# learner-shx/SVG-IR

Hardware: AMD Instinct MI355X
Metric: Gaussian-surfels/sec fwd+bwd @800x800 (1 view) (higher is better)
Workload: dtype f32; 1 GPU; cfg2: rgss path, P=200000 surfels, 800x800, SH degree 3, S=5, VS=0, fwd+bwd, one view per step per GPU (BASELINE.json configs[1] = cfg2 at N=1; configs[3] = cfg4, view r on rank r, at N>1); num_rendered=673008, parallelism=view-parallel x1, per_rank_cpus=not pinned

## Files before the change

### svg-ir_amd/csrc/api.hip

```cpp
#include <algorithm>
#include <cstdarg>
#include <cstdio>
#include <atomic>
#include <cstdlib>
#include <ctime>
#include <memory>
#include <mutex>
#include <string>
#include <vector>

#include "common.hpp"
#include "geom_bwd.hpp"
#include "workload_history.hpp"
#include "depth_sort_plan.hpp"

using namespace svgir;

namespace {

thread_local std::string g_err;
std::atomic<bool> g_prof{false};
WorkloadHistory g_history;
unsigned long long* pinned_words(size_t n) {
    void* ptr = nullptr;
    if (hipHostMalloc(&ptr, n * sizeof(unsigned long long), hipHostMallocCoherent) != hipSuccess) { (void)hipGetLastError(); return nullptr; }
    std::fill_n((unsigned long long*)ptr, n, 0ull);
    return (unsigned long long*)ptr;
}
unsigned long long* g_pinned = nullptr;
std::atomic<uint32_t> g_pinned_tag{0};
constexpr unsigned kPinnedSlots = 256;
std::once_flag g_pinned_once;
std::mutex g_pinned_mu;
uint64_t g_pinned_busy[kPinnedSlots / 64];
struct PinnedSlot {
    unsigned long long* at = nullptr; uint32_t tag = 0; int index = -1;
    PinnedSlot() {
        std::call_once(g_pinned_once, [] { g_pinned = pinned_words(2 * kPinnedSlots); });
        tag = ++g_pinned_tag;
        if (tag == 0) tag = ++g_pinned_tag;
        if (!g_pinned) return;
        static const unsigned usable = [] { const char* e = getenv("SVGIR_PINNED_SLOTS"); return e ? (unsigned)std::min<long>(std::max<long>(atol(e), 0), kPinnedSlots) : kPinnedSlots; }();
        std::lock_guard<std::mutex> lk(g_pinned_mu);
        for (unsigned i = 0; i < usable; i++)
            if (!(g_pinned_busy[i / 64] >> (i % 64) & 1ull)) {
                g_pinned_busy[i / 64] |= 1ull << (i % 64);
                index = (int)i;
                at = g_pinned + 2 * index;
                return;
            }
    }
    ~PinnedSlot() {
        if (index < 0) return;
        std::lock_guard<std::mutex> lk(g_pinned_mu);
        g_pinned_busy[index / 64] &= ~(1ull << (index % 64));
    }
    PinnedSlot(const PinnedSlot&) = delete;
    PinnedSlot& operator=(const PinnedSlot&) = delete;
};
double spin_budget_s() {
    static const double v = [] {
        const char* e = getenv("SVGIR_SPIN_MS");
        return e ? std::max(0.0, atof(e)) * 1e-3 : 0.05;
    }();
    return v;
}
inline bool tagged_pair(volatile unsigned long long* at, uint32_t tag, uint32_t* w0, uint32_t* w1) {
    const unsigned long long v0 = at[0], v1 = at[1];
    if ((uint32_t)(v0 >> 32) != tag || (uint32_t)(v1 >> 32) != tag) return false;
    *w0 = (uint32_t)v0; *w1 = (uint32_t)v1;
    return true;
}
bool pinned_spin(volatile unsigned long long* at, uint32_t tag, uint32_t* w0, uint32_t* w1) {
    struct timespec t0;
    clock_gettime(CLOCK_MONOTONIC, &t0);
    const double budget = spin_budget_s();
    for (long long spin = 0;; spin++) {
        if (tagged_pair(at, tag, w0, w1)) return true;
        if ((spin & 255) == 255 || budget == 0.0) {
            struct timespec t1;
            clock_gettime(CLOCK_MONOTONIC, &t1);
            const double el = (double)(t1.tv_sec - t0.tv_sec) + 1e-9 * (double)(t1.tv_nsec - t0.tv_nsec);
            if (el >= budget) return false;
            if (el > 5e-3) { struct timespec ts = {0, 20000}; nanosleep(&ts, nullptr); }
        }
    }
}
struct ViewEntry { const void* key = nullptr; uint32_t tag = 0; int cap_R = 0; long long cap_slots = -1; unsigned long long stamp = 0;
                   bool queue = false;
                   bool recorded = false;
                   hipStream_t stream = nullptr; };
constexpr int kViewEntries = 1024;
std::mutex g_view_mu;
ViewEntry g_view[kViewEntries];
constexpr int kViewWords = 4;
unsigned long long* g_view_pinned = nullptr;
unsigned long long g_view_clock = 0;
uint32_t g_view_tag = 0;
unsigned long long* view_note(const void* image_blob, int cap_R, long long cap_slots, bool queue, uint32_t* tag, hipStream_t stream) {
    std::lock_guard<std::mutex> lk(g_view_mu);
    if (!g_view_pinned && !(g_view_pinned = pinned_words(kViewEntries * kViewWords))) return nullptr;
    int slot = 0;
    for (int i = 0; i < kViewEntries; i++) {
        if (g_view[i].key == image_blob) { slot = i; break; }
        if (g_view[i].stamp < g_view[slot].stamp) slot = i;
    }
    ViewEntry& e = g_view[slot];
    e.key = image_blob; e.stamp = ++g_view_clock; e.cap_R = cap_R; e.cap_slots = cap_slots; e.recorded = false;
    e.stream = stream; e.queue = queue;
    e.tag = ++g_view_tag ? g_view_tag : ++g_view_tag;
    *tag = e.tag;
    return g_view_pinned + kViewWords * slot;
}
constexpr uint32_t kBlobMagic = 0x53564931u, kBlobMagicQueue = 0x53564932u;
struct ViewCounts { bool known = false; bool queue = false; int cap_R = 0; long long cap_slots = -1, pairs = -1, slots = -1, nonempty = -1; hipError_t err = hipSuccess; };
enum class Wait { kCaps, kLook, kBlock };
ViewCounts resolve_view(const void* image_blob, const uint32_t* blob_counters, Wait how, const hipStream_t* stream, bool caps = false,
                        const CapKey* record = nullptr) {
    ViewCounts out;
    if (!image_blob) return out;
    int i = 0;
    uint32_t tag = 0;
    hipStream_t fwd_stream = nullptr;
    {
        std::lock_guard<std::mutex> lk(g_view_mu);
        while (g_view_pinned && i < kViewEntries && g_view[i].key != image_blob) i++;
        if (!g_view_pinned || i == kViewEntries) i = -1;
        else { tag = g_view[i].tag; fwd_stream = g_view[i].stream; out.cap_R = g_view[i].cap_R; out.cap_slots = g_view[i].cap_slots; out.queue = g_view[i].queue; }
    }
    out.known = i >= 0;
    if (out.known && how != Wait::kCaps) {
        volatile unsigned long long* at = g_view_pinned + kViewWords * i;
        uint32_t w0 = 0, w1 = 0;
        bool got = how == Wait::kLook ? tagged_pair(at, tag, &w0, &w1) : pinned_spin(at, tag, &w0, &w1);
        if (!got && how == Wait::kBlock) {
            hipError_t e = hipErrorInvalidHandle;
            if (stream) e = hipStreamSynchronize(*stream);
            else {
                const hipError_t q = fwd_stream ? hipStreamQuery(fwd_stream) : hipSuccess;
                if (q == hipSuccess || q == hipErrorNotReady) e = hipStreamSynchronize(fwd_stream);
                else (void)hipGetLastError();
            }
            if (e != hipSuccess) { (void)hipGetLastError(); e = hipDeviceSynchronize(); }
            if (e != hipSuccess) (void)hipGetLastError();
            got = tagged_pair(at, tag, &w0, &w1);
        }
        if (got) {
            out.pairs = (long long)w0; out.slots = (long long)w1;
            const unsigned long long v2 = at[2];
            if ((uint32_t)(v2 >> 32) == tag) out.nonempty = (long long)(uint32_t)v2;
            bool first = false;
            if (record) {
                std::lock_guard<std::mutex> lk(g_view_mu);
                if (g_view[i].key == image_blob && !g_view[i].recorded) g_view[i].recorded = first = true;
            }
            if (first) g_history.record_slots(*record, out.slots, out.nonempty);
        }
    }
    if (blob_counters && (!out.known || (caps && out.cap_slots < 0) || (how != Wait::kCaps && out.pairs < 0))) {
        uint32_t w[8] = {0, 0, 0, 0, 0, 0, 0, 0};
        out.err = stream ? hipStreamSynchronize(*stream) : hipDeviceSynchronize();
        const bool read = out.err == hipSuccess && hipMemcpy(w, blob_counters, sizeof(w), hipMemcpyDeviceToHost) == hipSuccess;
        if (out.err == hipSuccess && !read) (void)hipGetLastError();
        if (!read || (w[3] != kBlobMagic && w[3] != kBlobMagicQueue)) return out;
        out.known = true; out.queue = w[3] == kBlobMagicQueue; out.pairs = (long long)w[1]; out.slots = (long long)w[2]; out.cap_R = (int)w[4];
        out.cap_slots = (long long)((unsigned long long)w[5] | ((unsigned long long)w[6] << 32));
    }
    return out;
}
struct SideStream { hipStream_t s = nullptr; bool ok = false; };
std::mutex g_side_mu;
SideStream g_side[16];
hipStream_t side_stream(hipStream_t of) {
    int dev = 0;
    hipDevice_t sd;
    if (of != nullptr && hipStreamGetDevice(of, &sd) == hipSuccess) dev = (int)sd;
    else if (hipGetDevice(&dev) != hipSuccess) return nullptr;
    if (dev < 0 || dev >= 16) return nullptr;
    std::lock_guard<std::mutex> lk(g_side_mu);
    SideStream& ss = g_side[dev];
    if (!ss.ok) {
        int least = 0, greatest = 0;
        (void)hipDeviceGetStreamPriorityRange(&least, &greatest);
        if (hipStreamCreateWithPriority(&ss.s, hipStreamNonBlocking, least) != hipSuccess) return nullptr;
        ss.ok = true;
    }
    return ss.s;
}
std::mutex g_times_mu;
struct Pending { hipEvent_t a, b; const char* name; };
std::vector<Pending> g_pending;
struct Accum { const char* name; double sum_ms; int count; };
std::vector<Accum> g_accum;

int fail(int code, const char* fmt, ...) {
    char buf[512];
    va_list ap;
    va_start(ap, fmt);
    vsnprintf(buf, sizeof(buf), fmt, ap);
    va_end(ap);
    g_err = buf;
    return code;
}

#define HIP_OK(expr)                                                                                   \
    do {                                                                                               \
        hipError_t e_ = (expr);                                                                        \
        if (e_ != hipSuccess) return fail(SVGIR_ERR_HIP, "%s failed: %s", #expr, hipGetErrorString(e_)); \
    } while (0)

void resolve_pending() {
    std::vector<Pending> todo;
    {
        std::lock_guard<std::mutex> lk(g_times_mu);
        todo.swap(g_pending);
    }
    std::vector<hipEvent_t> seen;
    for (auto& p : todo) {
        (void)hipEventSynchronize(p.b);
        float ms = 0.f;
        if (hipEventElapsedTime(&ms, p.a, p.b) == hipSuccess) {
            std::lock_guard<std::mutex> lk(g_times_mu);
            bool found = false;
            for (auto& acc : g_accum)
                if (acc.name == p.name) { acc.sum_ms += ms; acc.count++; found = true; break; }
            if (!found) g_accum.push_back({p.name, (double)ms, 1});
        }
        for (hipEvent_t e : {p.a, p.b}) {
            bool dup = false;
            for (auto x : seen) if (x == e) dup = true;
            if (!dup) seen.push_back(e);
        }
    }
    for (auto e : seen) (void)hipEventDestroy(e);
}

}

namespace svgir {
StageMarks stage_begin(hipStream_t s) {
    StageMarks t{s, g_prof.load(), nullptr};
    if (t.on) {
        if (hipEventCreate(&t.prev) != hipSuccess) t.on = false;
        else (void)hipEventRecord(t.prev, s);
    }
    return t;
}
void stage_mark(StageMarks& t, const char* name) {
    if (!t.on) return;
    hipEvent_t e;
    if (hipEventCreate(&e) != hipSuccess) { t.on = false; return; }
    (void)hipEventRecord(e, t.s);
    {
        std::lock_guard<std::mutex> lk(g_times_mu);
        g_pending.push_back({t.prev, e, name});
    }
    t.prev = e;
}
int report_error(int code, const char* fmt, ...) {
    char buf[512];
    va_list ap;
    va_start(ap, fmt);
    vsnprintf(buf, sizeof(buf), fmt, ap);
    va_end(ap);
    g_err = buf;
    return code;
}
}

namespace {

struct ViewGrid { int W, H, gx, gy, T; };
ViewGrid view_grid(int W, int H) {
    const int gx = (W + TILE - 1) / TILE, gy = (H + TILE - 1) / TILE;
    return {W, H, gx, gy, (int)((long long)gx * gy)};
}

CfgRef cfg_ref(const svgir_params* p) {
    CfgRef c;
    if (p->variant == SVGIR_SVGSS) { c.ptr = p->config; c.len = p->config ? p->config_len : 0; }
    else { c.ptr = nullptr; c.len = -1; }
    return c;
}

constexpr int kListMinP = 400000, kListMinPRows = 50000;

bool high_fill(long long nonempty) {
    static const int forced = [] { const char* e = getenv("SVGIR_FWD_FILL"); return e ? (atoi(e) != 0 ? 1 : 0) : -1; }();
    return forced >= 0 ? forced != 0 : nonempty >= 8192;
}

bool shade_prepass(int Ns) {
    static const int forced = [] { const char* e = getenv("SVGIR_PREPASS"); return e ? (atoi(e) != 0 ? 1 : 0) : -1; }();
    return forced >= 0 ? forced != 0 : Ns >= 128;
}

int validate(const svgir_params* p, bool fwd) {
    if (!p) return fail(SVGIR_ERR_INVALID, "params is NULL");
    if (p->variant != SVGIR_RGSS && p->variant != SVGIR_SVGSS) return fail(SVGIR_ERR_INVALID, "unknown variant %d", p->variant);
    if (p->P < 0 || p->W <= 0 || p->H <= 0) return fail(SVGIR_ERR_INVALID, "bad sizes P=%d W=%d H=%d", p->P, p->W, p->H);
    if (p->P > 40000000) return fail(SVGIR_ERR_INVALID, "P=%d exceeds the supported 40 000 000 Gaussians (32-bit byte offsets into the splat records)", p->P);
    const ViewGrid v = view_grid(p->W, p->H);
    if (v.gx > 1023 || v.gy > 1023 || 4ll * v.gx * v.gy >= (1ll << (32 - SEG_K_BITS)))
        return fail(SVGIR_ERR_INVALID, "image %dx%d exceeds the supported size (at most 1023 tiles per side, %lld tiles in total)",
                    p->W, p->H, (1ll << (32 - SEG_K_BITS)) / 4 - 1);
    if (p->P == 0) return 0;
    if (!p->means3D || !p->viewmatrix || !p->projmatrix || !p->background)
        return fail(SVGIR_ERR_INVALID, "means3D/viewmatrix/projmatrix/background must be provided");
    if (fwd && !p->opacities) return fail(SVGIR_ERR_INVALID, "opacities must be provided");
    if (!p->colors_precomp && !p->shs)
        return fail(SVGIR_ERR_INVALID, "For non-RGB, provide precomputed Gaussian colors!");
    if (p->shs && (p->D < 0 || p->D > 3 || p->M < (p->D + 1) * (p->D + 1)))
        return fail(SVGIR_ERR_INVALID, "SH degree %d needs M >= %d coefficients (M=%d)", p->D, (p->D + 1) * (p->D + 1), p->M);
    if (p->shs && !p->cam_pos) return fail(SVGIR_ERR_INVALID, "cam_pos is required with SHs");
    if (!p->cov3D_precomp && !(p->scales && p->rotations))
        return fail(SVGIR_ERR_INVALID, "provide scales+rotations or cov3D_precomp");
    if (p->S < 0 || (p->S > 0 && !p->features)) return fail(SVGIR_ERR_INVALID, "features missing for S=%d", p->S);
    if (p->variant == SVGIR_SVGSS) {
        if (p->VS < 0 || p->VS % 4 != 0) return fail(SVGIR_ERR_INVALID, "VS=%d must be a non-negative multiple of 4", p->VS);
        if (p->VS > 0 && !p->vfeatures) return fail(SVGIR_ERR_INVALID, "vfeatures missing for VS=%d", p->VS);
        if (!p->patchbbox) return fail(SVGIR_ERR_INVALID, "patchbbox is required for svgss");
        if (p->S > 50 || p->VS / 4 > 20) return fail(SVGIR_ERR_INVALID, "svgss supports S<=50, VS/4<=20 (Q9)");
    } else {
        if (p->VS != 0) return fail(SVGIR_ERR_INVALID, "rgss has no vfeatures");
        if (p->S > 33) return fail(SVGIR_ERR_INVALID, "rgss supports S<=33 (Q9)");
    }
    if (p->shade) {
        const svgir_shade_params& sp = p->shade->sp;
        if (p->variant != SVGIR_SVGSS) return fail(SVGIR_ERR_INVALID, "fused shading belongs to the svgss variant");
        if (sp.P != p->P) return fail(SVGIR_ERR_INVALID, "fused shading: sp.P = %d but P = %d", sp.P, p->P);
        if (p->S != (sp.training ? 4 : 7) || p->VS != (sp.training ? 52 : 64))
            return fail(SVGIR_ERR_INVALID, "fused shading packs S = %d, VS = %d (training = %d), not S = %d, VS = %d", sp.training ? 4 : 7,
                        sp.training ? 52 : 64, sp.training, p->S, p->VS);
        if (!sp.viewmatrix) return fail(SVGIR_ERR_INVALID, "fused shading needs sp.viewmatrix (packed view-space normals)");
    }
    return 0;
}

CapKey workload_key(const svgir_params* p) {
    int dev_id = 0;
    (void)hipGetDevice(&dev_id);
    return CapKey{dev_id, p->W, p->H, p->P, p->S, p->variant == SVGIR_SVGSS ? p->VS : 0, p->variant, p->workload_scope};
}

bool bin_capacity(size_t bytes, const char* image_blob, int W, int H, int nstate, Wait how, const hipStream_t* stream, ViewCounts* vc) {
    const bool compact = bin_bytes_compact(bytes);
    if (compact || how != Wait::kCaps)
        *vc = resolve_view(image_blob, image_layout(const_cast<char*>(image_blob), W, H).counters, how, stream, compact);
    if (compact) return vc->known && vc->cap_slots >= 0;
    vc->cap_R = binning_capacity_from_bytes(bytes, view_grid(W, H).T, nstate);
    vc->cap_slots = -1;
    return true;
}

template <class A> void camera_args(A& a, const svgir_params* p) {
    a.P = p->P; a.D = p->D; a.M = p->M; a.means3D = p->means3D; a.shs = p->colors_precomp ? nullptr : p->shs;
    a.scales = p->scales; a.rotations = p->rotations; a.view = p->viewmatrix; a.proj = p->projmatrix; a.campos = p->cam_pos;
    a.scale_modifier = p->scale_modifier; a.tanx = p->tan_fovx; a.tany = p->tan_fovy; a.cfg = cfg_ref(p);
    a.focal_x = p->W / (2.0f * p->tan_fovx); a.focal_y = p->H / (2.0f * p->tan_fovy);
}

RenderArgs render_args(const svgir_params* p, const ViewGrid& v, const GeomLayout& G, const ImageLayout& I, const BinLayout& B, int fin) {
    const bool svgss = p->variant == SVGIR_SVGSS;
    RenderArgs ra{};
    ra.W = v.W; ra.H = v.H; ra.gx = v.gx; ra.gy = v.gy; ra.S = p->S; ra.VS = svgss ? p->VS : 0;
    ra.ranges = I.ranges; ra.point_list = B.val[fin]; ra.rec = G.rec; ra.features = p->features; ra.vfeatures = p->vfeatures;
    ra.bg = p->background; ra.cfg = cfg_ref(p);
    ra.sub_list = B.sub_list; ra.sub_total = I.sub_total; ra.sub_order = I.sub_order; ra.sub_count = I.sub_count; ra.sub_ndump = I.sub_ndump;
    ra.sub_pair_base = I.sub_pair_base; ra.sub_slot_base = I.sub_slot_base; ra.disp_ctr = I.disp_ctr; ra.disp_item = I.disp_item;
    ra.seg_list = B.seg_list; ra.seg_desc = B.seg_desc; ra.seg_count = I.counters; ra.seg_block = I.seg_block; ra.seg_state = B.seg_state;
    ra.slot_cap = (uint32_t)std::min<size_t>(B.slot_cap, 0xffffffffu);
    ra.order_n = (int)order_entries(v.gx, v.gy);
    ra.bg_in_render = render_specialised(p->S, ra.VS, svgss) ? 1 : 0;
    ra.final_T = I.final_T; ra.final_D = I.final_D; ra.n_contrib = I.n_contrib;
    return ra;
}
}

extern "C" {

int svgir_abi_version(void) { return SVGIR_ABI_VERSION; }
size_t svgir_geom_bytes(int32_t P) { return geom_layout(nullptr, P).bytes; }
size_t svgir_image_bytes(int32_t W, int32_t H) { return image_layout(nullptr, W, H).bytes; }
size_t svgir_binning_bytes(int32_t R, int32_t W, int32_t H, int32_t S, int32_t VS) {
    return bin_layout(nullptr, binning_capacity(R), view_grid(W, H).T, seg_nstate(S, VS)).bytes;
}
size_t svgir_image_ncontrib_offset(int32_t W, int32_t H) { return image_layout(nullptr, W, H).ncontrib_off; }
size_t svgir_image_ranges_offset(int32_t W, int32_t H) {
    const ImageLayout I = image_layout((char*)256, W, H);
    return (size_t)((char*)I.ranges - (char*)256);
}
size_t svgir_binning_point_list_offset(size_t binning_bytes, const char* image_blob, int32_t W, int32_t H, int32_t S, int32_t VS) {
    const int T = view_grid(W, H).T, nstate = seg_nstate(S, VS);
    ViewCounts vc;
    if (!bin_capacity(binning_bytes, image_blob, W, H, nstate, Wait::kCaps, nullptr, &vc)) return (size_t)-1;
    const BinLayout B = bin_layout((char*)256, vc.cap_R, T, nstate);
    return (size_t)((char*)B.val[tile_sort_plan(T).passes & 1] - (char*)256);
}
const char* svgir_last_error(void) { return g_err.c_str(); }
void svgir_set_profiling(int enabled) {
    resolve_pending();
    if (enabled) {
        std::lock_guard<std::mutex> lk(g_times_mu);
        g_accum.clear();
    }
    g_prof.store(enabled != 0);
}
int svgir_last_timings(const char** names, float* avg_ms, int* counts, int cap) {
    resolve_pending();
    std::lock_guard<std::mutex> lk(g_times_mu);
    int n = 0;
    for (auto& acc : g_accum) {
        if (n >= cap) break;
        names[n] = acc.name;
        avg_ms[n] = (float)(acc.sum_ms / (acc.count > 0 ? acc.count : 1));
        if (counts) counts[n] = acc.count;
        n++;
    }
    return n;
}

struct ForwardCall {
    const svgir_view_call c; const svgir_params* p = c.params; const svgir_outputs* o = c.outputs; hipStream_t s = (hipStream_t)c.stream;
    bool key_spec;
    int P = 0, nstate = 0, fin = 0, spec_top = -1, cap = 0;
    ViewGrid v{};
    bool svgss = false, shade_subset = false, prepass = false, done = false;
    char *gblob = nullptr, *iblob = nullptr, *bblob = nullptr;
    GeomLayout G{}; ImageLayout I{}; TileSortPlan plan{};
    CapKey ckey{}; const uint32_t* depth_order = nullptr; long long cap_slots = -1;
    hipEvent_t features_ready = nullptr;
    PinnedSlot R_pin;
    StageMarks tm;

    ForwardCall(const svgir_view_call& c_, bool key_spec_) : c(c_), key_spec(key_spec_), tm(stage_begin(s)) {}

    int check(const char* what) {
        hipError_t e = p->debug ? hipStreamSynchronize(s) : hipSuccess;
        if (e == hipSuccess) e = hipGetLastError();
        return e != hipSuccess ? fail(SVGIR_ERR_HIP, p->debug ? "%s failed: %s" : "%s launch failed: %s", what, hipGetErrorString(e)) : 0;
    }

    int run_binning_and_render(char* bblob, int cap, long long cap_slots, bool timed, bool cull_only = false) {
        const BinLayout B = bin_layout(bblob, cap, v.T, nstate, cap_slots);
        launch_emit(P, depth_order, G.tiles, G.offsets, G.rec, o->radii, v.gx, v.gy, B.key[0], B.val[0], cap, I.ranges,
                    I.counters, B.radix_tbl, G.counters + 3, I.disp_ctr, s);
        if (int rc = check("emit")) return rc;
        if (timed) stage_mark(tm, "emit");
        if (plan.single) {
            launch_tile_sort12(B.key, B.val, cap, G.counters, B.radix_tbl, I.ranges, v.T, s);
            if (int rc = check("tile sort")) return rc;
            if (timed) stage_mark(tm, "sort_tile");
        } else {
            launch_radix_sort(B.key, B.val, cap, G.counters, plan.bits, plan.bits_per_pass, B.radix_tbl, s);
            if (int rc = check("tile sort")) return rc;
            if (timed) stage_mark(tm, "sort_tile");
            launch_ranges(cap, G.counters, B.key[fin], I.ranges, v.T, s);
            if (int rc = check("ranges")) return rc;
            if (timed) stage_mark(tm, "ranges");
        }

        RenderArgs ra = render_args(p, v, G, I, B, fin);
        ra.hi_fill = high_fill(g_history.guess_fill(ckey)) ? 1 : 0;
        ra.out_color = o->out_color; ra.out_normal = o->out_normal; ra.out_depth = o->out_depth; ra.out_opacity = o->out_opacity;
        ra.out_feature = o->out_feature; ra.out_vfeature = o->out_vfeature; ra.out_weights = o->out_weights;
        const bool clear_stencil = !svgss && !p->computer_pseudo_normal;
        ra.zero_a = clear_stencil ? o->out_pseudo_normal : nullptr;
        ra.zero_b = clear_stencil ? o->out_surface_xyz : nullptr;
        static const int xcd_forced = [] { const char* e = getenv("SVGIR_FWD_XCD"); return e ? (atoi(e) != 0 ? 1 : 0) : -1; }();
        const bool per_xcd = ra.bg_in_render && (xcd_forced >= 0 ? xcd_forced != 0 : ra.hi_fill != 0);
        uint32_t vtag = 0;
        unsigned long long* vslot = view_note(iblob, cap, cap_slots, !per_xcd, &vtag, s);
        ra.queue_order = per_xcd ? 0 : 1;
        ra.pub_host = vslot; ra.pub_tag = vtag; ra.pub_cap_R = (uint32_t)cap; ra.pub_cap_slots = cap_slots; ra.pub_magic = kBlobMagicQueue;
        ra.publish = ra.queue_order;
        launch_cull(ra, s);
        if (per_xcd) {
            const bool row_path = svgss && p->VS > 0 && render_specialised(p->S, p->VS, true);
            launch_order_desc(I.sub_total, 4 * v.T, I.sub_order, row_path ? I.sub_pair_base : nullptr, I.sub_slot_base, I.counters, vslot, vtag,
                              (uint32_t)cap, cap_slots, kBlobMagic, v.gx, ra.order_n, s);
        } else if (cull_only) {
            launch_dispatch_publish(ra, s);
        }
        if (int rc = check("cull")) return rc;
        if (timed) stage_mark(tm, "cull");
        if (cull_only) return 0;
        if (prepass) {
            RenderArgs rp = ra;
            ra.publish = 0;
            rp.S = 0; rp.VS = 0; rp.features = nullptr; rp.vfeatures = nullptr; rp.needed = G.needed;
            launch_contrib_prepass(rp, s);
            if (int rc = check("prepass")) return rc;
            if (timed) stage_mark(tm, "prepass");
        }
        if (p->shade) {
            svgir_shade_params sp = p->shade->sp;
            sp.subset = nullptr; sp.subset_count = nullptr;
            if (prepass) {
                uint32_t* cnt = G.shade_work + partition_work_words(P) - 1;
                launch_partition(P, G.needed, nullptr, G.shade_list, G.shade_work, cnt, s);
                sp.subset = G.shade_list; sp.subset_count = cnt;
            } else if (shade_subset) {
                sp.subset = depth_order; sp.subset_count = G.counters + 3;
            }
            if (shade_forward_impl(&sp, p->shade->reduced, const_cast<float*>(p->features), const_cast<float*>(p->vfeatures), true, s) != 0)
                return fail(SVGIR_ERR_INVALID, "fused shading: svgir_shade_forward rejected its parameters");
            if (int rc = check("shade")) return rc;
            if (timed) stage_mark(tm, "shade");
        }
        if (features_ready && hipStreamWaitEvent(s, features_ready, 0) != hipSuccess) return fail(SVGIR_ERR_HIP, "waiting for the features event");
        if (launch_render_fwd(ra, svgss, s) < 0) launch_render_fwd_generic(ra, svgss, s);
        if (int rc = check("render")) return rc;
        if (timed) stage_mark(tm, "render");
        return 0;
    }

    int begin() {
        if (int rc = validate(p, true)) return rc;
        features_ready = (hipEvent_t)p->features_ready;
        if (!o || !c.geom || !c.binning || !c.image) return fail(SVGIR_ERR_INVALID, "outputs / allocators must be provided");
        P = p->P; v = view_grid(p->W, p->H);
        svgss = p->variant == SVGIR_SVGSS;
        if (P == 0) {
            const size_t N = (size_t)v.W * v.H;
            HIP_OK(hipMemsetAsync(o->out_color, 0, 3 * N * 4, s));
            HIP_OK(hipMemsetAsync(o->out_normal, 0, 3 * N * 4, s));
            HIP_OK(hipMemsetAsync(o->out_depth, 0, N * 4, s));
            HIP_OK(hipMemsetAsync(o->out_opacity, 0, N * 4, s));
            if (p->S) HIP_OK(hipMemsetAsync(o->out_feature, 0, (size_t)p->S * N * 4, s));
            if (svgss && p->VS) HIP_OK(hipMemsetAsync(o->out_vfeature, 0, (size_t)(p->VS / 4) * N * 4, s));
            if (!svgss && o->out_pseudo_normal) HIP_OK(hipMemsetAsync(o->out_pseudo_normal, 0, 3 * N * 4, s));
            if (!svgss && o->out_surface_xyz) HIP_OK(hipMemsetAsync(o->out_surface_xyz, 0, 3 * N * 4, s));
            done = true;
            return 1;
        }
        gblob = c.geom(geom_layout(nullptr, P).bytes, c.geom_ctx);
        iblob = c.image(image_layout(nullptr, v.W, v.H).bytes, c.image_ctx);
        if (!gblob || !iblob) return fail(SVGIR_ERR_ALLOC, "geometry/image blob allocation failed");
        G = geom_layout(gblob, P);
        I = image_layout(iblob, v.W, v.H);

        PreArgs pa;
        camera_args(pa, p);
        pa.W = v.W; pa.H = v.H; pa.gx = v.gx; pa.gy = v.gy; pa.colors_precomp = p->colors_precomp; pa.opacities = p->opacities;
        pa.cov3D_precomp = p->cov3D_precomp; pa.patchbbox = p->patchbbox;
        pa.rec = G.rec; pa.cov3D = G.cov3D; pa.clamped = G.clamped; pa.tiles = G.tiles; pa.key = G.key[0]; pa.idx = G.idx[0];
        pa.radii = o->radii;
        pa.out_weights = o->out_weights;
        pa.features = nullptr; pa.embed_S = 0;
        if (rec_embeds_features(p->S, svgss ? p->VS : 0)) {
            if (features_ready && hipStreamWaitEvent(s, features_ready, 0) != hipSuccess) return fail(SVGIR_ERR_HIP, "waiting for the features event");
            features_ready = nullptr; pa.features = p->features; pa.embed_S = p->S; }
        shade_subset = p->shade && !p->shade->all_surfels;
        prepass = shade_subset && shade_prepass(p->shade->sp.Ns);
        pa.needed = prepass ? G.needed : nullptr;
        pa.span = G.counters + 3;
        if (p->shade) pa.tabs = shade_tables(&p->shade->sp, nullptr, 0);
        pa.zero_words = radix_gtot(G.radix_tbl, P); pa.n_zero_words = (int)radix_gtot_words(P);
        ckey = workload_key(p);
        static const bool key_spec_env = getenv("SVGIR_NO_KEY_SPEC") == nullptr;
        spec_top = (key_spec && key_spec_env) ? g_history.guess_top(ckey) : -1;
        pa.spec_top = spec_top; pa.key_top = G.key_top;
        pa.prefilter_violation = nullptr;
        if (p->prefiltered) {
            HIP_OK(hipMemsetAsync(G.counters, 0, 16, s));
            pa.prefilter_violation = G.counters + 1;
        }
        launch_preprocess(pa, svgss, s);
        if (int rc = check("preprocess")) return rc;
        stage_mark(tm, "preprocess");

        const int depth_bits = spec_top >= 0 ? 24 : 32;
        depth_order = G.idx[(depth_bits / 8) & 1];
        const RadixWeights rw{G.tiles, G.radix_wtbl, G.offsets, G.counters, G.key_top, (P + 63) / 64, pa.prefilter_violation, R_pin.at, R_pin.tag};
        static const bool forced_lsd = depth_sort_forced_lsd(getenv("SVGIR_DEPTH_SORT"));
        static const int bucket_cap = depth_bucket_cap(getenv("SVGIR_DEPTH_BUCKET_CAP"));
        if (depth_sort_plan(P, spec_top, forced_lsd) == DepthSortPlan::kBuckets) launch_depth_bucket_sort(G.key, G.idx, P, G.radix_tbl, bucket_cap, s, rw);
        else launch_radix_sort(G.key, G.idx, P, nullptr, depth_bits, 8, G.radix_tbl, s, &rw);
        if (int rc = check("depth sort")) return rc;
        stage_mark(tm, "sort_depth");

        nstate = seg_nstate(p->S, svgss ? p->VS : 0);
        plan = tile_sort_plan(v.T);
        fin = plan.passes & 1;

        cap = 0; cap_slots = -1; bblob = nullptr;
        CapKey pkey = ckey;
        (void)resolve_view(g_history.last_view(ckey, &pkey.P), nullptr, Wait::kLook, nullptr, false, &pkey);
        long long gs = -1;
        if (const int guess = g_history.guess(ckey, &gs)) {
            cap = binning_capacity((long long)guess + guess / 8 + 1024);
            cap_slots = p->forward_only ? 0 : (gs < 0 ? -1 : std::min<long long>(gs + gs / 8 + 64, (long long)seg_capacity(cap, v.T)));
            bblob = c.binning(bin_layout(nullptr, cap, v.T, nstate, cap_slots).bytes, c.binning_ctx);
            if (bblob) {
                if (int rc = run_binning_and_render(bblob, cap, cap_slots, true)) return rc;
            } else {
                cap = 0;
            }
        }
        return 0;
    }

    static int run(const svgir_view_call& c, bool key_spec) {
        ForwardCall f(c, key_spec);
        const int rc = f.begin();
        return rc != 0 ? (rc < 0 ? rc : 0) : f.finish();
    }

    int finish() {
        if (done) return 0;
        done = true;
        uint32_t R_host = 0, R_aux = 0;
        bool have_R = R_pin.at && pinned_spin(R_pin.at, R_pin.tag, &R_host, &R_aux);
        if (!have_R) {
            const hipError_t e = hipStreamSynchronize(s);
            if (e != hipSuccess) return fail(SVGIR_ERR_HIP, "the forward failed on the device: %s", hipGetErrorString(e));
            have_R = R_pin.at && tagged_pair(R_pin.at, R_pin.tag, &R_host, &R_aux);
            if (!have_R) {
                uint32_t w[3] = {0, 0, 0};
                HIP_OK(hipMemcpy(w, G.counters, 12, hipMemcpyDeviceToHost));
                R_host = w[0]; R_aux = ((p->prefiltered && w[1]) ? 1u << 16 : 0u) | (w[2] & 0xffffu);
            }
        }
        if (p->prefiltered && (R_aux >> 16) != 0u) {
            (void)hipStreamSynchronize(s);
            return fail(SVGIR_ERR_INVALID, "Point is filtered although prefiltered is set. This shouldn't happen!");
        }
        if (R_host > 0x7ffff000u) return fail(SVGIR_ERR_INVALID, "instance count %u overflows int32", R_host);
        const int R = (int)R_host;
        {
            const uint32_t summary = R_aux & 0xffffu;
            if (key_spec) { g_history.record_top(ckey, summary); g_history.count(WorkloadHistory::kForwards); }
            if (spec_top >= 0) g_history.count(WorkloadHistory::kThreePass);
            const int av = (int)((summary >> 8) & 0xffu), ov = (int)(summary & 0xffu);
            if (spec_top >= 0 && !(av == 0xff && ov == 0) && (av != spec_top || ov != spec_top)) {
                HIP_OK(hipStreamSynchronize(s));
                g_history.count(WorkloadHistory::kRerunTop);
                return run(c, false);
            }
        }
        g_history.record_R(ckey, R);
        if (!bblob || R > cap) {
            const bool redo = bblob != nullptr;
            if (redo) { HIP_OK(hipStreamSynchronize(s)); g_history.count(WorkloadHistory::kRerunR); }
            cap = binning_capacity(R);
            cap_slots = p->forward_only ? 0 : -1;
            if (cap_slots < 0 && R > 0) {
                void* tmp = nullptr;
                if (hipMallocAsync(&tmp, bin_layout(nullptr, cap, v.T, nstate, 0).bytes, s) == hipSuccess) {
                    const int rc = run_binning_and_render((char*)tmp, cap, 0, false, true);
                    const ViewCounts vc = rc == 0 ? resolve_view(iblob, nullptr, Wait::kBlock, &s) : ViewCounts{};
                    (void)hipFreeAsync(tmp, s);
                    if (rc) return rc;
                    if (vc.slots >= 0) cap_slots = std::min<long long>(vc.slots, (long long)seg_capacity(cap, v.T));
                } else {
                    (void)hipGetLastError();
                }
            }
            bblob = c.binning(bin_layout(nullptr, cap, v.T, nstate, cap_slots).bytes, c.binning_ctx);
            if (!bblob) return fail(SVGIR_ERR_ALLOC, "binning blob allocation failed");
            if (redo && o->out_weights) HIP_OK(hipMemsetAsync(o->out_weights, 0, (size_t)P * 4, s));
            if (int rc = run_binning_and_render(bblob, cap, cap_slots, !redo)) return rc;
        }
        g_history.set_last_view(ckey, iblob, P);

        if (!svgss && p->computer_pseudo_normal) {
            launch_image_ops(v.W, v.H, p->viewmatrix, v.W / (2.0f * p->tan_fovx), v.H / (2.0f * p->tan_fovy), p->cx, p->cy, o->out_opacity,
                             o->out_depth, o->out_pseudo_normal, o->out_surface_xyz, s);
            if (int rc = check("image ops")) return rc;
            stage_mark(tm, "image");
        }
        return R;
    }
};

struct BackwardCall {
    const svgir_params* p; const svgir_grads* g; int R; const int32_t* radii; char *geom_blob, *binning_blob; size_t binning_bytes;
    char *image_blob, *scratch; size_t scratch_bytes; hipStream_t s;
    ViewCounts caps;
    ViewGrid v{};
    bool svgss = false;
    GeomLayout G{}; ImageLayout I{}; BinLayout B{};
    RenderArgs ra{};
    StageMarks tm{};
    RenderBwdArgs ba{};
    bool generic = false, rows = false, clear_in_kernel = false;
    ShadeTables shade_tabs;
    const uint32_t* blended = nullptr; const uint32_t* blended_n = nullptr;
    struct FreeAsync { void* p; hipStream_t s; ~FreeAsync() { if (p) (void)hipFreeAsync(p, s); } } redump{nullptr, s};
    struct ClearJoin {
        hipStream_t s; hipEvent_t ev = nullptr;
        void join() {
            if (ev) { (void)hipStreamWaitEvent(s, ev, 0); (void)hipEventDestroy(ev); ev = nullptr; }
        }
        ~ClearJoin() { join(); }
    } cleared{s};

    bool in_clear_region(const float* t, size_t floats) const {
        const char* b = (const char*)g->clear_base, *q = (const char*)t;
        return b && q >= b && q + floats * 4 <= b + g->clear_bytes;
    }

    int run() {
        if (int rc = locate()) return rc < 0 ? rc : 0;
        tm = stage_begin(s);
        if (int rc = redump_states()) return rc;
        if (int rc = clears()) return rc;
        if (int rc = seg_build()) return rc;
        composite();
        grad_reduce();
        if (int rc = shade_backward()) return rc;
        return geom_backward();
    }

    int locate() {
        if (int rc = validate(p, false)) return rc;
        if (p->P == 0) return 1;
        if (!g || !radii || !geom_blob || !binning_blob || !image_blob)
            return fail(SVGIR_ERR_INVALID, "grads / radii / blobs must be provided");
        if (p->shade) {
            if (!g->dL_dbase_color || !g->dL_droughness || !g->dL_dshade_normals || (!g->dL_dradiance && !p->shade->sp.radiance_ratio) || !g->dL_denv ||
                !g->env_grad_work)
                return fail(SVGIR_ERR_INVALID, "fused shading: the gradient outputs of the shading inputs must be provided");
            if (!render_specialised(p->S, p->VS, true)) return fail(SVGIR_ERR_INVALID, "fused shading without a specialised composite");
            if (g->dL_dreduced && !p->shade->all_surfels) return fail(SVGIR_ERR_INVALID, "fused shading: dL_dreduced needs all_surfels");
            if (!p->shade->all_surfels && !g->out_weights) return fail(SVGIR_ERR_INVALID, "fused shading: out_weights (the forward's) must be provided");
            if (g->dL_dviewdirs && in_clear_region(g->dL_dviewdirs, 3 * (size_t)p->P) != in_clear_region(g->dL_dbase_color, 12 * (size_t)p->P))
                return fail(SVGIR_ERR_INVALID, "fused shading: dL_dviewdirs must lie inside clear_base together with the per-surfel shading gradients, or outside together with them");
        } else if (g->dL_dviewdirs) {
            return fail(SVGIR_ERR_INVALID, "dL_dviewdirs needs the fused shading (svgir_params.shade)");
        }
        v = view_grid(p->W, p->H);
        svgss = p->variant == SVGIR_SVGSS;
        G = geom_layout(geom_blob, p->P);
        I = image_layout(image_blob, v.W, v.H);
        const int nstate = seg_nstate(p->S, svgss ? p->VS : 0);
        if (!bin_capacity(binning_bytes, image_blob, v.W, v.H, nstate, Wait::kCaps, &s, &caps)) {
            if (caps.err != hipSuccess) return fail(SVGIR_ERR_HIP, "hipStreamSynchronize(s) failed: %s", hipGetErrorString(caps.err));
            return fail(SVGIR_ERR_INVALID, "the binning blob (%zu bytes) has a compact layout, but the image blob does not describe it "
                                           "(not the image blob of the same svgir_forward?)", binning_bytes);
        }
        if (caps.cap_R < R || bin_layout(nullptr, caps.cap_R, v.T, nstate, caps.cap_slots).bytes != binning_bytes)
            return fail(SVGIR_ERR_INVALID, "binning blob of %zu bytes does not match any layout for R=%d", binning_bytes, R);
        B = bin_layout(binning_blob, caps.cap_R, v.T, nstate, caps.cap_slots);
        ra = render_args(p, v, G, I, B, tile_sort_plan(v.T).passes & 1);
        ba.W = ra.W; ba.H = ra.H; ba.gx = ra.gx; ba.gy = ra.gy; ba.S = ra.S; ba.VS = ra.VS;
        ba.ranges = ra.ranges; ba.point_list = ra.point_list; ba.rec = ra.rec; ba.features = ra.features; ba.vfeatures = ra.vfeatures;
        ba.bg = ra.bg; ba.cfg = ra.cfg; ba.sub_list = ra.sub_list; ba.sub_count = ra.sub_count; ba.sub_ndump = ra.sub_ndump;
        ba.seg_list = ra.seg_list; ba.seg_desc = ra.seg_desc; ba.seg_count = ra.seg_count; ba.seg_state = ra.seg_state;
        ba.final_T = ra.final_T; ba.final_D = ra.final_D; ba.n_contrib = ra.n_contrib;
        ba.seg_cap = (int)B.seg_cap;
        ba.backward_geometry = p->backward_geometry;
        ba.g_color = g->dL_dout_color; ba.g_normal = g->dL_dout_normal; ba.g_depth = g->dL_dout_depth;
        ba.g_opacity = g->dL_dout_opacity; ba.g_feature = g->dL_dout_feature; ba.g_vfeature = g->dL_dout_vfeature;
        ba.dL_dmean2D = g->dL_dmeans2D; ba.dL_dconic = g->dL_dconic; ba.dL_dopacity = g->dL_dopacity; ba.dL_dcolor = g->dL_dcolors;
        ba.dL_dfeature = g->dL_dfeatures; ba.dL_dvfeature = g->dL_dvfeatures; ba.dL_dnormal = g->dL_dnormal; ba.dL_ddepth = g->dL_ddepth;
        generic = !render_specialised(p->S, ba.VS, svgss);
        rows = ba.VS > 0 && !generic;
        ba.grad_rows = generic ? nullptr : (float*)scratch;
        if (rows && scratch) {
            ba.row_of = (uint32_t*)scratch;
            ba.grad_rows = (float*)(scratch + grad_rowof_bytes(caps.cap_R));
            ba.rows_cap = (uint32_t)std::min<size_t>((scratch_bytes - grad_rowof_bytes(caps.cap_R)) / ((size_t)grad_row_geom(p->S, ba.VS).RS * 4),
                                                     0xfffffff0u);
        }
        return 0;
    }

    int redump_states() {
        const bool verify = caps.cap_slots >= 0 && R > 0;
        const CapKey ckey = workload_key(p);
        const ViewCounts vc = resolve_view(image_blob, verify ? I.counters : nullptr, Wait::kBlock, &s, false, &ckey);
        if (verify && vc.slots < 0) {
            if (vc.err != hipSuccess) return fail(SVGIR_ERR_HIP, "hipStreamSynchronize(s) failed: %s", hipGetErrorString(vc.err));
            return fail(SVGIR_ERR_INVALID, "the image blob does not carry this view's state-slot total (forward failed, or a foreign blob)");
        }
        const long long slots = verify ? vc.slots : -1;
        static const bool trace = getenv("SVGIR_TRACE_SPEC") != nullptr;
        if (trace) fprintf(stderr, "[svgir] backward: R=%d capacity=%d state slots: capacity %lld, view %lld%s\n", R, caps.cap_R, caps.cap_slots, slots, (verify && slots > caps.cap_slots) ? " -> re-dump" : "");
        if (!verify || slots <= caps.cap_slots) return 0;
        if (!render_specialised(p->S, svgss ? p->VS : 0, svgss)) return fail(SVGIR_ERR_INVALID, "state slots without a specialised composite");
        HIP_OK(hipMallocAsync(&redump.p, align_up((size_t)slots * seg_nstate(p->S, ra.VS) * 64 * 4), s));
        ba.seg_state = ra.seg_state = (float*)redump.p;
        g_history.count(WorkloadHistory::kRerunSlots);
        RenderArgs rd = ra;
        rd.slot_cap = (uint32_t)std::min<long long>(slots, 0xffffffffll);
        rd.dump_only = 1;
        rd.queue_order = vc.queue ? 1 : 0;
        if (launch_render_fwd(rd, svgss, s) < 0) return fail(SVGIR_ERR_INVALID, "state re-dump: no specialised composite");
        stage_mark(tm, "state_redump");
        return 0;
    }

    int clears() {
        const size_t need = svgir_backward_scratch_bytes_for(p->variant, p->P, binning_bytes, image_blob, v.W, v.H, p->S, ba.VS);
        if (!generic && (!scratch || scratch_bytes < need))
            return fail(SVGIR_ERR_INVALID, "backward scratch of %zu bytes is smaller than svgir_backward_scratch_bytes_for() = %zu",
                        scratch ? scratch_bytes : (size_t)0, need);
        clear_in_kernel = !generic && R > 0 && g->clear_base && g->clear_bytes && (((uintptr_t)g->clear_base | g->clear_bytes) & 15) == 0;
        ba.clear = clear_in_kernel ? (uint4*)g->clear_base : nullptr;
        ba.clear_n16 = clear_in_kernel ? g->clear_bytes / 16 : 0;
        if (!clear_in_kernel) {
            hipStream_t cs = generic ? s : side_stream(s);
            if (!cs) cs = s;
            hipEvent_t ev_fork = nullptr;
            if (cs != s) {
                HIP_OK(hipEventCreateWithFlags(&ev_fork, hipEventDisableTiming));
                HIP_OK(hipEventRecord(ev_fork, s));
                HIP_OK(hipStreamWaitEvent(cs, ev_fork, 0));
                (void)hipEventDestroy(ev_fork);
            }
            const size_t Pz = (size_t)p->P * 4;
            if (g->clear_base && g->clear_bytes) {
                HIP_OK(hipMemsetAsync(g->clear_base, 0, g->clear_bytes, cs));
            } else {
                struct { float* p; size_t n; } t[] = {
                    {g->dL_dmeans2D, 3 * Pz}, {g->dL_dconic, 4 * Pz}, {g->dL_dopacity, Pz}, {g->dL_dcolors, 3 * Pz},
                    {g->dL_dfeatures, (size_t)p->S * Pz}, {g->dL_dvfeatures, (size_t)ba.VS * Pz}, {g->dL_dnormal, 3 * Pz},
                    {g->dL_ddepth, Pz}, {g->dL_dmeans3D, 3 * Pz}, {g->dL_dcov3D, 6 * Pz}, {g->dL_dsh, (size_t)p->M * 3 * Pz},
                    {g->dL_dscales, 3 * Pz}, {g->dL_drotations, 4 * Pz}, {svgss ? g->dL_dviewmat : nullptr, 64},
                    {svgss ? g->dL_dprojmat : nullptr, 64}, {svgss ? g->dL_dcampos : nullptr, 12}};
                for (auto& e : t)
                    if (e.p && e.n) HIP_OK(hipMemsetAsync(e.p, 0, e.n, cs));
            }
            if (cs != s) {
                HIP_OK(hipEventCreateWithFlags(&cleared.ev, hipEventDisableTiming));
                HIP_OK(hipEventRecord(cleared.ev, cs));
            }
        }
        return 0;
    }

    int seg_build() {
        void* sc_clear = rows ? (void*)ba.row_of : (void*)ba.grad_rows;
        const size_t sc_bytes = rows ? grad_rowof_bytes(caps.cap_R) : align_up((size_t)p->P * packed_row_geom(p->S).RS * 4);
        bool use_list = false;
        if (R > 0) {
            if (p->shade && g->env_grad_work) shade_tabs = shade_tables(&p->shade->sp, g->env_grad_work, p->shade->sp.env_h * p->shade->sp.env_w * 3);
            use_list = g->out_weights && !generic && (p->shade || p->P >= (rows ? kListMinPRows : kListMinP));
            launch_seg_build(ra, sc_clear, sc_bytes, shade_tabs, use_list ? g->out_weights : nullptr, p->P, G.shade_work, s);
        } else if (sc_clear && !rows) {
            HIP_OK(hipMemsetAsync(sc_clear, 0, sc_bytes, s));
        }
        stage_mark(tm, "seg_build");
        if (use_list && R > 0) {
            uint32_t* cnt = G.shade_work + partition_work_words(p->P) - 1;
            launch_partition_scatter(p->P, g->out_weights, G.shade_list, G.shade_work, cnt, s);
            blended = G.shade_list; blended_n = cnt;
        }
        return 0;
    }

    void composite() {
        if (R > 0) {
            if (generic) launch_render_bwd_generic(ba, svgss, s);
            else (void)launch_render_bwd(ba, svgss, s);
        }
        stage_mark(tm, "render_bwd");
        cleared.join();
    }

    void grad_reduce() {
        if (!(R > 0 && rows)) return;
        GradReduceArgs ga;
        ga.list = blended; ga.list_count = blended_n;
        ga.P = p->P; ga.S = p->S; ga.VS = ba.VS; ga.radii = radii; ga.tiles = G.tiles; ga.rec = G.rec;
        ga.grad_rows = ba.grad_rows; ga.row_of = ba.row_of;
        ga.dL_dmean2D = g->dL_dmeans2D; ga.dL_dconic = g->dL_dconic; ga.dL_dopacity = g->dL_dopacity; ga.dL_dcolor = g->dL_dcolors;
        ga.dL_dfeature = g->dL_dfeatures; ga.dL_dvfeature = g->dL_dvfeatures; ga.dL_dnormal = g->dL_dnormal; ga.dL_ddepth = g->dL_ddepth;
        launch_grad_reduce(ga, s);
        stage_mark(tm, "grad_reduce");
    }

    int shade_backward() {
        if (!p->shade) return 0;
        const bool all = p->shade->all_surfels != 0;
        svgir_shade_params sp = p->shade->sp;
        sp.subset = nullptr; sp.subset_count = nullptr;
        if (!all) {
            if (!blended) {
                uint32_t* cnt = G.shade_work + partition_work_words(p->P) - 1;
                launch_partition(p->P, nullptr, g->out_weights, G.shade_list, G.shade_work, cnt, s);
                blended = G.shade_list; blended_n = cnt;
            }
            sp.subset = blended; sp.subset_count = blended_n;
        }
        auto in_clear = [&](const float* t, size_t floats) {
            const char* b = (const char*)g->clear_base, *q = (const char*)t;
            return clear_in_kernel && q >= b && q + floats * 4 <= b + g->clear_bytes;
        };
        const size_t Pz = (size_t)p->P;
        const bool precleared = in_clear(g->dL_dbase_color, 12 * Pz) && in_clear(g->dL_droughness, 4 * Pz) &&
                                in_clear(g->dL_dshade_normals, 12 * Pz) &&
                                (!g->dL_dradiance || in_clear(g->dL_dradiance, 3 * Pz * (size_t)sp.Ns)) &&
                                (!g->dL_dviewdirs || in_clear(g->dL_dviewdirs, 3 * Pz));
        if (shade_backward_impl(&sp, g->dL_dreduced, g->dL_dfeatures, g->dL_dvfeatures, g->dL_dbase_color, g->dL_droughness,
                                g->dL_dshade_normals, g->dL_dradiance, g->dL_denv, g->env_grad_work, g->dL_dradiance_ratio, g->dL_dviewdirs, precleared,
                                shade_tabs.env != nullptr, s) != 0)
            return fail(SVGIR_ERR_INVALID, "fused shading: svgir_shade_backward rejected its parameters");
        stage_mark(tm, "shade_bwd");
        return 0;
    }

    int geom_backward() {
        GeomBwdArgs ga;
        ga.list = R > 0 ? blended : nullptr; ga.list_count = blended_n;
        camera_args(ga, p);
        ga.cov3D = p->cov3D_precomp ? p->cov3D_precomp : G.cov3D; ga.radii = radii; ga.clamped = G.clamped; ga.svgss = svgss;
        ga.dL_dmean2D = g->dL_dmeans2D; ga.dL_dconic = g->dL_dconic; ga.dL_dcolor = g->dL_dcolors; ga.dL_dnormal = g->dL_dnormal;
        ga.dL_ddepth = g->dL_ddepth;
        ga.packed = (rows || generic) ? nullptr : ba.grad_rows; ga.S = p->S;
        ga.dL_dopacity = g->dL_dopacity; ga.dL_dfeature = g->dL_dfeatures;
        ga.dL_dmean3D = g->dL_dmeans3D; ga.dL_dcov3D = g->dL_dcov3D; ga.dL_dsh = g->dL_dsh; ga.dL_dscale = g->dL_dscales;
        ga.dL_drot = g->dL_drotations; ga.dL_dviewmat = g->dL_dviewmat; ga.dL_dprojmat = g->dL_dprojmat; ga.dL_dcampos = g->dL_dcampos;
        if (ga.scales && !ga.rotations) return fail(SVGIR_ERR_INVALID, "rotations missing");
        launch_geom_bwd_blended(ga, g->out_weights, s);
        stage_mark(tm, "geom_bwd");
        hipError_t e = p->debug ? hipStreamSynchronize(s) : hipSuccess;
        if (e == hipSuccess) e = hipGetLastError();
        return e != hipSuccess ? fail(SVGIR_ERR_HIP, "backward failed: %s", hipGetErrorString(e)) : 0;
    }
};

int svgir_forward(const svgir_params* p, const svgir_outputs* o, svgir_alloc_fn geom, void* geom_ctx,
                  svgir_alloc_fn binning, void* binning_ctx, svgir_alloc_fn image, void* image_ctx, void* stream) {
    return ForwardCall::run({p, o, geom, geom_ctx, binning, binning_ctx, image, image_ctx, stream, 0}, true);
}

int svgir_forward_batch(svgir_view_call* views, int32_t count) {
    if (count < 0 || (count > 0 && !views)) return fail(SVGIR_ERR_INVALID, "views is NULL");
    std::vector<std::unique_ptr<ForwardCall>> calls;
    calls.reserve((size_t)count);
    int first_err = 0;
    for (int v = 0; v < count; v++) {
        calls.emplace_back(new ForwardCall(views[v], true));
        const int rc = calls.back()->begin();
        views[v].num_rendered = rc < 0 ? rc : 0;
        if (rc < 0 && !first_err) first_err = rc;
    }
    const std::string begin_err = first_err ? g_err : std::string();
    for (int v = 0; v < count; v++) {
        if (views[v].num_rendered < 0) continue;
        const int rc = calls[(size_t)v]->finish();
        views[v].num_rendered = rc;
        if (rc < 0 && !first_err) first_err = rc;
    }
    if (!begin_err.empty()) g_err = begin_err;
    return first_err;
}
void svgir_reset_workload_history(int32_t scope) { g_history.reset(scope); }
void svgir_speculation_stats(int64_t* out5) {
    if (out5) g_history.stats(out5);
}

size_t svgir_backward_scratch_bytes(int32_t variant, int32_t P, size_t binning_bytes, int32_t W, int32_t H, int32_t S,
                                    int32_t VS) {
    return svgir_backward_scratch_bytes_for(variant, P, binning_bytes, nullptr, W, H, S, VS);
}

size_t svgir_backward_scratch_bytes_for(int32_t variant, int32_t P, size_t binning_bytes, const char* image_blob, int32_t W, int32_t H,
                                        int32_t S, int32_t VS) {
    if (!render_specialised(S, variant == SVGIR_SVGSS ? VS : 0, variant == SVGIR_SVGSS))
        return 256;
    if (variant != SVGIR_SVGSS || VS == 0)
        return align_up((size_t)(P > 0 ? P : 1) * packed_row_geom(S).RS * 4);
    ViewCounts vc;
    if (!bin_capacity(binning_bytes, image_blob, W, H, seg_nstate(S, VS), Wait::kBlock, nullptr, &vc))
        vc.cap_R = binning_capacity((long long)(binning_bytes / 48));
    if (image_blob && vc.pairs < 0) (void)hipGetLastError();
    const size_t rows = vc.pairs >= 0 ? (size_t)std::min<long long>(vc.pairs, (long long)4 * vc.cap_R) : (size_t)4 * vc.cap_R;
    return grad_scratch_bytes(vc.cap_R, rows > 0 ? rows : 1, S, VS);
}

int svgir_backward(const svgir_params* p, const svgir_grads* g, int32_t R, const int32_t* radii, char* geom_blob,
                   char* binning_blob, size_t binning_bytes, char* image_blob, char* scratch, size_t scratch_bytes,
                   void* stream) {
    return BackwardCall{p, g, R, radii, geom_blob, binning_blob, binning_bytes, image_blob, scratch, scratch_bytes, (hipStream_t)stream}.run();
}

int svgir_mark_visible(int32_t variant, int32_t P, const float* means3D, const float* viewmatrix,
                       const float* projmatrix, uint8_t* present, void* stream) {
    (void)projmatrix;
    if (P < 0) return fail(SVGIR_ERR_INVALID, "P < 0");
    if (P == 0 || variant == SVGIR_SVGSS) return 0;
    if (!means3D || !viewmatrix || !present) return fail(SVGIR_ERR_INVALID, "NULL pointer");
    launch_mark_visible(P, means3D, viewmatrix, present, (hipStream_t)stream);
    hipError_t e = hipGetLastError();
    if (e != hipSuccess) return fail(SVGIR_ERR_HIP, "mark_visible failed: %s", hipGetErrorString(e));
    return 0;
}

}
```

### svg-ir_amd/csrc/binning.hip

```cpp
#include <algorithm>
#include <cassert>

#include "common.hpp"
#include "depth_sort_plan.hpp"

namespace svgir {

namespace {

constexpr int GS = 32;

__device__ __forceinline__ uint32_t key_top_fold(uint32_t a, uint32_t b) { return (a & b & 0xff00u) | ((a | b) & 0xffu); }

struct WeightArgs {
    const uint32_t* vals;
    uint32_t* wgtot;
    RadixWeights w;
};

template <int ITEMS, bool W = false, bool F = false>
__global__ void __launch_bounds__(BLOCK) radix_hist_kernel(const uint32_t* __restrict__ keys, int n_cap,
                                                           const uint32_t* __restrict__ n_dev, int bit_lo,
                                                           uint32_t mask, uint32_t* __restrict__ table,
                                                           uint32_t* __restrict__ gtot, WeightArgs wa) {
    __shared__ uint32_t hist[256];
    __shared__ uint32_t whist[W ? 256 : 1];
    const int n = n_dev ? (int)min((uint32_t)n_cap, n_dev[0]) : n_cap;
    hist[threadIdx.x] = 0;
    if constexpr (W) whist[threadIdx.x] = 0;
    __syncthreads();
    const int base = blockIdx.x * (BLOCK * ITEMS);
    uint32_t k[ITEMS];
#pragma unroll
    for (int i = 0; i < ITEMS; i++) k[i] = keys[max(0, min(base + i * BLOCK + (int)threadIdx.x, n - 1))];
    uint32_t w[W ? ITEMS : 1];
    if constexpr (W) {
        uint32_t g[ITEMS];
#pragma unroll
        for (int i = 0; i < ITEMS; i++) g[i] = wa.vals[max(0, min(base + i * BLOCK + (int)threadIdx.x, n - 1))];
#pragma unroll
        for (int i = 0; i < ITEMS; i++) w[i] = wa.w.tiles[2 * (size_t)g[i]];
    }
#pragma unroll
    for (int i = 0; i < ITEMS; i++) {
        const int e = base + i * BLOCK + threadIdx.x;
        if constexpr (F) { if (e < n && w[i] != 0u) atomicAdd(&hist[(k[i] >> bit_lo) & mask], 1u); }
        else if (e < n) atomicAdd(&hist[(k[i] >> bit_lo) & mask], 1u);
        if constexpr (W) if (e < n && w[i] != 0u) atomicAdd(&whist[(k[i] >> bit_lo) & mask], w[i]);
    }
    __syncthreads();
    const uint32_t c = hist[threadIdx.x];
    table[(size_t)blockIdx.x * 256 + threadIdx.x] = c;
    if (c) atomicAdd(&gtot[(size_t)(blockIdx.x / GS) * 256 + threadIdx.x], c);
    if constexpr (W) {
        const uint32_t wc = whist[threadIdx.x];
        if constexpr (!F) wa.w.wtable[(size_t)blockIdx.x * 256 + threadIdx.x] = wc;
        if (wc) atomicAdd(&wa.wgtot[(size_t)(blockIdx.x / GS) * 256 + threadIdx.x], wc);
    }
}

template <int ITEMS, bool W = false>
__global__ void __launch_bounds__(BLOCK) radix_scatter_kernel(const uint32_t* __restrict__ kin,
                                                              const uint32_t* __restrict__ vin,
                                                              uint32_t* __restrict__ kout, uint32_t* __restrict__ vout,
                                                              int n_cap, const uint32_t* __restrict__ n_dev, int bit_lo, int nbits,
                                                              const uint32_t* __restrict__ table,
                                                              const uint32_t* __restrict__ gtot, int ngroups, WeightArgs wa) {
    __shared__ uint32_t wcnt[4][256];
    __shared__ uint32_t wtot[4];
    __shared__ uint32_t wtot2[W ? 4 : 1], ksum[W ? 4 : 1], smax[W ? 4 : 1];
    const int t = threadIdx.x, lane = t & 63, wave = t >> 6;
    const uint32_t mask = (1u << nbits) - 1;
    const int n = n_dev ? (int)min((uint32_t)n_cap, n_dev[0]) : n_cap;
    const int base = blockIdx.x * (BLOCK * ITEMS) + wave * (64 * ITEMS);
    const unsigned long long lt_mask = (lane == 0) ? 0ull : (~0ull >> (64 - lane));
    uint32_t ks[ITEMS], vs[ITEMS], rk[ITEMS];
#pragma unroll
    for (int c = 0; c < ITEMS; c++) {
        const int e = base + c * 64 + lane;
        ks[c] = e < n ? kin[e] : 0u;
        vs[c] = e < n ? vin[e] : 0u;
    }
    uint32_t ws[W ? ITEMS : 1];
    if constexpr (W) {
#pragma unroll
        for (int c = 0; c < ITEMS; c++) ws[c] = base + c * 64 + lane < n ? wa.w.tiles[2 * (size_t)vs[c]] : 0u;
        if (blockIdx.x == 0) {
            uint32_t kv = 0xff00u;
#pragma unroll 8
            for (int j = t; j < wa.w.n_key_top; j += BLOCK) kv = key_top_fold(kv, wa.w.key_top[j]);
            kv = wave_reduce(kv, key_top_fold);
            if (lane == 0) ksum[wave] = kv;
        }
    }
#pragma unroll
    for (int w = 0; w < 4; w++) wcnt[w][t] = 0;
    uint32_t cursor;
    uint32_t wcursor = 0;
    {
        const int g = blockIdx.x / GS;
        uint32_t tot = 0, pre = 0, wsum = 0, wpre = 0;
#pragma unroll 8
        for (int gg = 0; gg < ngroups; gg++) {
            const uint32_t v = gtot[(size_t)gg * 256 + t];
            tot += v;
            pre += gg < g ? v : 0u;
            if constexpr (W) {
                const uint32_t wv = wa.wgtot[(size_t)gg * 256 + t];
                wsum += wv;
                wpre += gg < g ? wv : 0u;
            }
        }
#pragma unroll 8
        for (int b = g * GS; b < (int)blockIdx.x; b++) {
            pre += table[(size_t)b * 256 + t];
            if constexpr (W) wpre += wa.w.wtable[(size_t)b * 256 + t];
        }
        cursor = block_excl_scan<4>(tot, wtot) + pre;
        if constexpr (W) {
            uint32_t R;
            wcursor = block_excl_scan<4>(wsum, wtot2, &R) + wpre;
            if (blockIdx.x == 0 && t == 0) {
                const uint32_t summary = key_top_fold(key_top_fold(ksum[0], ksum[1]), key_top_fold(ksum[2], ksum[3]));
                wa.w.counters[0] = R;
                wa.w.counters[2] = summary;
                if (wa.w.host_out) {
                    const uint32_t viol = wa.w.violation ? (wa.w.violation[0] != 0u ? 1u : 0u) : 0u;
                    __hip_atomic_store(wa.w.host_out, ((unsigned long long)wa.w.host_tag << 32) | R, __ATOMIC_RELAXED, __HIP_MEMORY_SCOPE_SYSTEM);
                    __hip_atomic_store(wa.w.host_out + 1, ((unsigned long long)wa.w.host_tag << 32) | (viol << 16) | summary, __ATOMIC_RELAXED,
                                       __HIP_MEMORY_SCOPE_SYSTEM);
                }
            }
        }
    }
#pragma unroll
    for (int c = 0; c < ITEMS; c++) {
        const bool valid = base + c * 64 + lane < n;
        const uint32_t d = (ks[c] >> bit_lo) & mask;
        const unsigned long long same = wave_match(d, nbits, valid);
        const uint32_t in_round = (uint32_t)__popcll(same & lt_mask);
        const uint32_t prior = wcnt[wave][d];
        rk[c] = prior + in_round;
        if (valid && in_round == 0) wcnt[wave][d] = prior + (uint32_t)__popcll(same);
    }
    __syncthreads();
    if constexpr (W) {
        __shared__ uint32_t sV[BLOCK * ITEMS];
        __shared__ __attribute__((aligned(16))) uint32_t sS[BLOCK * ITEMS];
        __shared__ uint8_t sD[BLOCK * ITEMS];
        __shared__ uint32_t bstart[256], gcur[256], wgcur[256];
        const uint32_t c0 = wcnt[0][t], c1 = wcnt[1][t], c2 = wcnt[2][t], c3 = wcnt[3][t];
        const uint32_t bs = block_excl_scan<4>(c0 + c1 + c2 + c3, wtot);
        bstart[t] = bs; gcur[t] = cursor; wgcur[t] = wcursor;
        wcnt[0][t] = bs; wcnt[1][t] = bs + c0; wcnt[2][t] = bs + c0 + c1; wcnt[3][t] = bs + c0 + c1 + c2;
        __syncthreads();
        uint32_t span = 0;
#pragma unroll
        for (int c = 0; c < ITEMS; c++) {
            if (base + c * 64 + lane < n) {
                const uint32_t d = (ks[c] >> bit_lo) & mask;
                const uint32_t lp = wcnt[wave][d] + rk[c];
                sV[lp] = vs[c]; sS[lp] = ws[c]; sD[lp] = (uint8_t)d;
                if (ws[c] != 0u) span = max(span, gcur[d] + (lp - bstart[d]) + 1u);
            }
        }
        span = wave_reduce_max(span);
        if (lane == 0) smax[wave] = span;
        __syncthreads();
        const int nblk = min(BLOCK * ITEMS, n - (int)blockIdx.x * (BLOCK * ITEMS));
        uint32_t wv[ITEMS], sum = 0;
#pragma unroll
        for (int c = 0; c < ITEMS; c += 4) {
            const uint4 q = reinterpret_cast<const uint4*>(sS)[(t * ITEMS + c) >> 2];
            wv[c] = q.x; wv[c + 1] = q.y; wv[c + 2] = q.z; wv[c + 3] = q.w;
        }
#pragma unroll
        for (int c = 0; c < ITEMS; c++) { wv[c] = t * ITEMS + c < nblk ? wv[c] : 0u; sum += wv[c]; }
        uint32_t run = block_excl_scan<4>(sum, wtot2);
#pragma unroll
        for (int c = 0; c < ITEMS; c += 4) {
            uint4 q;
            q.x = run; run += wv[c]; q.y = run; run += wv[c + 1]; q.z = run; run += wv[c + 2]; q.w = run; run += wv[c + 3];
            reinterpret_cast<uint4*>(sS)[(t * ITEMS + c) >> 2] = q;
        }
        if (t == 0) {
            const uint32_t m = max(max(smax[0], smax[1]), max(smax[2], smax[3]));
            if (m != 0u) atomicMax(wa.w.counters + 3, m);
        }
        __syncthreads();
#pragma unroll
        for (int c = 0; c < ITEMS; c++) {
            const int i = c * BLOCK + t;
            if (i < nblk) {
                const uint32_t d = sD[i], b = bstart[d];
                const uint32_t pos = gcur[d] + ((uint32_t)i - b);
                vout[pos] = sV[i];
                wa.w.offsets[pos] = wgcur[d] + (sS[i] - sS[b]);
            }
        }
        return;
    }
    if (ITEMS >= 16) {
        __shared__ uint32_t sK[BLOCK * (ITEMS >= 16 ? ITEMS : 1)], sV[BLOCK * (ITEMS >= 16 ? ITEMS : 1)];
        __shared__ uint32_t bstart[256], gcur[256];
        const uint32_t c0 = wcnt[0][t], c1 = wcnt[1][t], c2 = wcnt[2][t], c3 = wcnt[3][t];
        const uint32_t bc = c0 + c1 + c2 + c3;
        const uint32_t bs = block_excl_scan<4>(bc, wtot);
        bstart[t] = bs; gcur[t] = cursor;
        wcnt[0][t] = bs; wcnt[1][t] = bs + c0; wcnt[2][t] = bs + c0 + c1; wcnt[3][t] = bs + c0 + c1 + c2;
        __syncthreads();
#pragma unroll
        for (int c = 0; c < ITEMS; c++) {
            if (base + c * 64 + lane < n) {
                const uint32_t lp = wcnt[wave][(ks[c] >> bit_lo) & mask] + rk[c];
                sK[lp] = ks[c]; sV[lp] = vs[c];
            }
        }
        __syncthreads();
        const int nblk = min(BLOCK * ITEMS, n - (int)blockIdx.x * (BLOCK * ITEMS));
#pragma unroll
        for (int c = 0; c < ITEMS; c++) {
            const int i = c * BLOCK + t;
            if (i < nblk) {
                const uint32_t k = sK[i], d = (k >> bit_lo) & mask;
                const uint32_t pos = gcur[d] + ((uint32_t)i - bstart[d]);
                kout[pos] = k;
                vout[pos] = sV[i];
            }
        }
        return;
    }
    {
        const uint32_t c0 = wcnt[0][t], c1 = wcnt[1][t], c2 = wcnt[2][t];
        __syncthreads();
        wcnt[0][t] = cursor; wcnt[1][t] = cursor + c0; wcnt[2][t] = cursor + c0 + c1; wcnt[3][t] = cursor + c0 + c1 + c2;
    }
    __syncthreads();
#pragma unroll
    for (int c = 0; c < ITEMS; c++) {
        if (base + c * 64 + lane < n) {
            const uint32_t pos = wcnt[wave][(ks[c] >> bit_lo) & mask] + rk[c];
            kout[pos] = ks[c];
            vout[pos] = vs[c];
        }
    }
}


template <int ITEMS>
__global__ void __launch_bounds__(BLOCK) depth_bucket_scatter_kernel(const uint32_t* __restrict__ kin, const uint32_t* __restrict__ vin,
                                                                     uint32_t* __restrict__ kout, uint32_t* __restrict__ vout,
                                                                     uint32_t* __restrict__ wout, int n, int bit_lo,
                                                                     const uint32_t* __restrict__ table, const uint32_t* __restrict__ gtot,
                                                                     const uint32_t* __restrict__ wgtot, int ngroups, RadixWeights w) {
    __shared__ uint32_t wcnt[4][256];
    __shared__ uint32_t wtot[4], wtot2[4], wtot3[4], ksum[4], wcul[4];
    const int t = threadIdx.x, lane = t & 63, wave = t >> 6;
    const int base = blockIdx.x * (BLOCK * ITEMS) + wave * (64 * ITEMS);
    const unsigned long long lt_mask = (lane == 0) ? 0ull : (~0ull >> (64 - lane));
    uint32_t ks[ITEMS], vs[ITEMS], ws[ITEMS], rk[ITEMS];
#pragma unroll
    for (int c = 0; c < ITEMS; c++) {
        const int e = base + c * 64 + lane;
        ks[c] = e < n ? kin[e] : 0u;
        vs[c] = e < n ? vin[e] : 0u;
    }
#pragma unroll
    for (int c = 0; c < ITEMS; c++) ws[c] = base + c * 64 + lane < n ? w.tiles[2 * (size_t)vs[c]] : 0u;
    if (blockIdx.x == 0) {
        uint32_t kv = 0xff00u;
#pragma unroll 8
        for (int j = t; j < w.n_key_top; j += BLOCK) kv = key_top_fold(kv, w.key_top[j]);
        kv = wave_reduce(kv, key_top_fold);
        if (lane == 0) ksum[wave] = kv;
    }
#pragma unroll
    for (int q = 0; q < 4; q++) wcnt[q][t] = 0;
    uint32_t cursor, nvis, cull_base;
    {
        const int g = blockIdx.x / GS;
        uint32_t tot = 0, pre = 0, wsum = 0;
#pragma unroll 8
        for (int gg = 0; gg < ngroups; gg++) {
            const uint32_t v = gtot[(size_t)gg * 256 + t];
            tot += v;
            pre += gg < g ? v : 0u;
            if (blockIdx.x == 0) wsum += wgtot[(size_t)gg * 256 + t];
        }
#pragma unroll 8
        for (int b = g * GS; b < (int)blockIdx.x; b++) pre += table[(size_t)b * 256 + t];
        cursor = block_excl_scan<4>(tot, wtot, &nvis) + pre;
        cull_base = nvis + blockIdx.x * (BLOCK * ITEMS) - block_sum<4>(pre, wtot3);
        if (blockIdx.x == 0) {
            uint32_t R;
            (void)block_excl_scan<4>(wsum, wtot2, &R);
            if (t == 0) {
                const uint32_t summary = key_top_fold(key_top_fold(ksum[0], ksum[1]), key_top_fold(ksum[2], ksum[3]));
                w.counters[0] = R;
                w.counters[2] = summary;
                w.counters[3] = nvis;
                if (w.host_out) {
                    const uint32_t viol = w.violation ? (w.violation[0] != 0u ? 1u : 0u) : 0u;
                    __hip_atomic_store(w.host_out, ((unsigned long long)w.host_tag << 32) | R, __ATOMIC_RELAXED, __HIP_MEMORY_SCOPE_SYSTEM);
                    __hip_atomic_store(w.host_out + 1, ((unsigned long long)w.host_tag << 32) | (viol << 16) | summary, __ATOMIC_RELAXED,
                                       __HIP_MEMORY_SCOPE_SYSTEM);
                }
            }
        }
    }
    uint32_t ncul = 0;
#pragma unroll
    for (int c = 0; c < ITEMS; c++) {
        const bool valid = base + c * 64 + lane < n && ws[c] != 0u;
        const uint32_t d = (ks[c] >> bit_lo) & 255u;
        const unsigned long long same = wave_match(d, 8, valid);
        const uint32_t in_round = (uint32_t)__popcll(same & lt_mask);
        const uint32_t prior = wcnt[wave][d];
        rk[c] = prior + in_round;
        if (valid && in_round == 0) wcnt[wave][d] = prior + (uint32_t)__popcll(same);
        const unsigned long long culled = __ballot(base + c * 64 + lane < n && ws[c] == 0u);
        if (!valid) rk[c] = ncul + (uint32_t)__popcll(culled & lt_mask);
        ncul += (uint32_t)__popcll(culled);
    }
    if (lane == 0) wcul[wave] = ncul;
    __syncthreads();
    {
        const uint32_t c0 = wcnt[0][t], c1 = wcnt[1][t], c2 = wcnt[2][t];
        __syncthreads();
        wcnt[0][t] = cursor; wcnt[1][t] = cursor + c0; wcnt[2][t] = cursor + c0 + c1; wcnt[3][t] = cursor + c0 + c1 + c2;
    }
    __syncthreads();
    for (int q = 0; q < wave; q++) cull_base += wcul[q];
#pragma unroll
    for (int c = 0; c < ITEMS; c++) {
        if (base + c * 64 + lane >= n) continue;
        if (ws[c] != 0u) {
            const uint32_t pos = wcnt[wave][(ks[c] >> bit_lo) & 255u] + rk[c];
            kout[pos] = ks[c];
            vout[pos] = vs[c];
            wout[pos] = ws[c];
        } else {
            vout[cull_base + rk[c]] = vs[c];
        }
    }
}

constexpr int DB_THREADS = 1024, DB_WAVES = DB_THREADS / 64, DB_ROUNDS = DEPTH_BUCKET_CAP / DB_THREADS;

template <bool CARRY, class Get, class Put>
__device__ __forceinline__ void bucket_pass(int m, int shift, Get get, Put put, uint32_t (*wcnt)[256], uint32_t* cur, uint32_t* wsum) {
    const int t = threadIdx.x, lane = t & 63, wave = t >> 6;
    const unsigned long long lt_mask = (lane == 0) ? 0ull : (~0ull >> (64 - lane));
    for (int i = t; i < DB_WAVES * 256; i += DB_THREADS) (&wcnt[0][0])[i] = 0u;
    __syncthreads();
    const int per = ((m + DB_WAVES - 1) / DB_WAVES + 63) & ~63;
    const int base = wave * per;
    uint2 it[DB_ROUNDS];
    uint32_t rk[DB_ROUNDS];
#pragma unroll
    for (int r = 0; r < DB_ROUNDS; r++) {
        if (r * 64 < per) {
            const int i = base + r * 64 + lane;
            const bool valid = i < m;
            it[r] = valid ? get(i) : make_uint2(0u, 0u);
            const uint32_t d = (it[r].x >> shift) & 255u;
            const unsigned long long same = wave_match(d, 8, valid);
            const uint32_t in_round = (uint32_t)__popcll(same & lt_mask);
            const uint32_t prior = wcnt[wave][d];
            rk[r] = prior + in_round;
            if (valid && in_round == 0) wcnt[wave][d] = prior + (uint32_t)__popcll(same);
        }
    }
    __syncthreads();
    uint32_t c[DB_WAVES], total = 0;
#pragma unroll
    for (int q = 0; q < DB_WAVES; q++) { c[q] = t < 256 ? wcnt[q][t] : 0u; total += c[q]; }
    uint32_t run;
    if constexpr (CARRY) run = t < 256 ? cur[t] : 0u;
    else run = block_excl_scan<DB_WAVES>(total, wsum);
    if (t < 256) {
#pragma unroll
        for (int q = 0; q < DB_WAVES; q++) { wcnt[q][t] = run; run += c[q]; }
        if constexpr (CARRY) cur[t] = run;
    }
    __syncthreads();
#pragma unroll
    for (int r = 0; r < DB_ROUNDS; r++) {
        if (r * 64 < per) {
            const int i = base + r * 64 + lane;
            if (i < m) put(wcnt[wave][(it[r].x >> shift) & 255u] + rk[r], it[r]);
        }
    }
    __syncthreads();
}

__global__ void __launch_bounds__(DB_THREADS) depth_bucket_sort_kernel(uint32_t* key0, uint32_t* val0, uint32_t* key1, uint32_t* val1, uint32_t* offsets,
                                                                       const uint32_t* __restrict__ tiles, const uint32_t* __restrict__ gtot,
                                                                       const uint32_t* __restrict__ wgtot, int ngroups, int cap) {
    __shared__ uint32_t sA[DEPTH_BUCKET_CAP], sB[DEPTH_BUCKET_CAP], sI[DEPTH_BUCKET_CAP], sW[DEPTH_BUCKET_CAP];
    __shared__ uint32_t wcnt[DB_WAVES][256];
    __shared__ uint32_t cur[256], wsum[DB_WAVES], wsum2[DB_WAVES], hdr[3], red[2][DB_WAVES];
    const int t = threadIdx.x, lane = t & 63, wave = t >> 6;
    uint32_t cnt = 0, wt = 0;
    if (t < 256)
        for (int g = 0; g < ngroups; g++) { cnt += gtot[(size_t)g * 256 + t]; wt += wgtot[(size_t)g * 256 + t]; }
    const uint32_t cpre = block_excl_scan<DB_WAVES>(cnt, wsum);
    const uint32_t wpre = block_excl_scan<DB_WAVES>(wt, wsum2);
    if (t == (int)blockIdx.x) { hdr[0] = cpre; hdr[1] = cnt; hdr[2] = wpre; }
    __syncthreads();
    const uint32_t start = hdr[0], wbase = hdr[2];
    const int n = (int)hdr[1];
    if (n == 0) return;
    if (n <= cap) {
        for (int i = t; i < n; i += DB_THREADS) {
            sA[i] = (key1[start + i] << 16) | (uint32_t)i;
            sI[i] = val1[start + i];
            sW[i] = offsets[start + i];
        }
        bucket_pass<false>(n, 16, [&](int i) { return make_uint2(sA[i], 0u); }, [&](uint32_t pos, uint2 it) { sB[pos] = it.x; }, wcnt, cur, wsum);
        bucket_pass<false>(n, 24, [&](int i) { return make_uint2(sB[i], 0u); }, [&](uint32_t pos, uint2 it) { sA[pos] = it.x; }, wcnt, cur, wsum);
        uint32_t wv[DB_ROUNDS], sum = 0;
#pragma unroll
        for (int j = 0; j < DB_ROUNDS; j++) {
            const int i = t * DB_ROUNDS + j;
            wv[j] = i < n ? sW[sA[i] & 0xffffu] : 0u;
            sum += wv[j];
        }
        uint32_t run = block_excl_scan<DB_WAVES>(sum, wsum2);
#pragma unroll
        for (int j = 0; j < DB_ROUNDS; j++) {
            const int i = t * DB_ROUNDS + j;
            if (i < n) sB[i] = run;
            run += wv[j];
        }
        __syncthreads();
        for (int i = t; i < n; i += DB_THREADS) {
            val1[start + i] = sI[sA[i] & 0xffffu];
            offsets[start + i] = wbase + sB[i];
        }
        return;
    }
    {
        uint32_t a = 0xffffu, o = 0u;
        for (int i = t; i < n; i += DB_THREADS) { const uint32_t k = key1[start + i] & 0xffffu; a &= k; o |= k; }
        a = wave_reduce(a, [](uint32_t x, uint32_t y) { return x & y; });
        o = wave_reduce(o, [](uint32_t x, uint32_t y) { return x | y; });
        if (lane == 0) { red[0][wave] = a; red[1][wave] = o; }
        __syncthreads();
        a = 0xffffu; o = 0u;
#pragma unroll
        for (int q = 0; q < DB_WAVES; q++) { a &= red[0][q]; o |= red[1][q]; }
        if (a != o) {
            for (int pass = 0; pass < 2; pass++) {
                const uint32_t* sk = (pass ? key0 : key1) + start; const uint32_t* sv = (pass ? val0 : val1) + start;
                uint32_t* dk = (pass ? key1 : key0) + start; uint32_t* dv = (pass ? val1 : val0) + start;
                const int shift = 8 * pass;
                if (t < 256) cur[t] = 0u;
                __syncthreads();
                for (int i = t; i < n; i += DB_THREADS) atomicAdd(&cur[(sk[i] >> shift) & 255u], 1u);
                __syncthreads();
                const uint32_t ex = block_excl_scan<DB_WAVES>(t < 256 ? cur[t] : 0u, wsum);
                if (t < 256) cur[t] = ex;
                for (int c0 = 0; c0 < n; c0 += cap)
                    bucket_pass<true>(min(cap, n - c0), shift, [&](int i) { return make_uint2(sk[c0 + i], sv[c0 + i]); },
                                      [&](uint32_t pos, uint2 it) { dk[pos] = it.x; dv[pos] = it.y; }, wcnt, cur, wsum);
                __threadfence_block();
                __syncthreads();
            }
        }
    }
    uint32_t carry = wbase;
    for (int c0 = 0; c0 < n; c0 += DB_THREADS * DB_ROUNDS) {
        uint32_t wv[DB_ROUNDS], sum = 0;
#pragma unroll
        for (int j = 0; j < DB_ROUNDS; j++) {
            const int i = c0 + t * DB_ROUNDS + j;
            wv[j] = i < n ? tiles[2 * (size_t)val1[start + i]] : 0u;
            sum += wv[j];
        }
        uint32_t all;
        uint32_t run = carry + block_excl_scan<DB_WAVES>(sum, wsum, &all);
#pragma unroll
        for (int j = 0; j < DB_ROUNDS; j++) {
            const int i = c0 + t * DB_ROUNDS + j;
            if (i < n) offsets[start + i] = run;
            run += wv[j];
        }
        carry += all;
        __syncthreads();
    }
}

#ifndef TS12_THREADS_V
#define TS12_THREADS_V 512
#endif
constexpr int TS12T = TS12_THREADS_V, TS12W = TS12T / 64, TS12K = 8 * TS12T;
static_assert(TS12K >= TS12_KEYS && TS12_BINS % TS12T == 0, "common.hpp tile12_table_words sizes the table for rows of TS12_KEYS keys");
__host__ __device__ constexpr int ts12_blocks(int n) { return (n + TS12K - 1) / TS12K; }
__global__ void __launch_bounds__(TS12T) ts12_hist_kernel(const uint32_t* __restrict__ keys, int n_cap, const uint32_t* __restrict__ n_dev,
                                                          uint32_t* __restrict__ table, int nbins) {
    __shared__ uint32_t hist[TS12_BINS];
    const int n = n_dev ? (int)min((uint32_t)n_cap, n_dev[0]) : n_cap;
    if ((int)blockIdx.x >= ts12_blocks(n)) return;
    const int t = threadIdx.x;
    for (int i = t; i < nbins; i += TS12T) hist[i] = 0u;
    __syncthreads();
    const int base = blockIdx.x * TS12K;
    uint32_t k[TS12K / TS12T];
#pragma unroll
    for (int i = 0; i < TS12K / TS12T; i++) k[i] = keys[max(0, min(base + i * TS12T + t, n - 1))];
#pragma unroll
    for (int i = 0; i < TS12K / TS12T; i++)
        if (base + i * TS12T + t < n) atomicAdd(&hist[k[i] & (TS12_BINS - 1)], 1u);
    __syncthreads();
    uint32_t* row = table + (size_t)blockIdx.x * nbins;
    for (int i = t; i < nbins; i += TS12T) row[i] = hist[i];
}

__global__ void __launch_bounds__(BLOCK) ts12_colscan_kernel(uint32_t* __restrict__ table, int nb_cap, int n_cap, const uint32_t* __restrict__ n_dev,
                                                             uint32_t* __restrict__ totals, int nbins) {
    __shared__ uint32_t psum[16][17];
    const int nb = n_dev ? (int)min((uint32_t)nb_cap, (uint32_t)ts12_blocks((int)min((uint32_t)n_cap, n_dev[0]))) : nb_cap;
    const int col = threadIdx.x & 15, seg = threadIdx.x >> 4;
    const int d = blockIdx.x * 16 + col;
    const int rps = (nb + 15) / 16, r0 = min(nb, seg * rps), r1 = min(nb, r0 + rps);
    uint32_t* colp = table + d;
    uint32_t sum = 0;
    int r = r0;
    for (; r + 8 <= r1; r += 8) {
        uint32_t c[8];
#pragma unroll
        for (int j = 0; j < 8; j++) c[j] = colp[(size_t)(r + j) * nbins];
#pragma unroll
        for (int j = 0; j < 8; j++) sum += c[j];
    }
    for (; r < r1; r++) sum += colp[(size_t)r * nbins];
    psum[seg][col] = sum;
    __syncthreads();
    uint32_t run = 0, all = 0;
#pragma unroll
    for (int sg = 0; sg < 16; sg++) { const uint32_t v = psum[sg][col]; run += sg < seg ? v : 0u; all += v; }
    if (seg == 0) totals[d] = all;
    r = r0;
    for (; r + 8 <= r1; r += 8) {
        uint32_t c[8];
#pragma unroll
        for (int j = 0; j < 8; j++) c[j] = colp[(size_t)(r + j) * nbins];
#pragma unroll
        for (int j = 0; j < 8; j++) { colp[(size_t)(r + j) * nbins] = run; run += c[j]; }
    }
    for (; r < r1; r++) { const uint32_t c = colp[(size_t)r * nbins]; colp[(size_t)r * nbins] = run; run += c; }
}

__global__ void __launch_bounds__(TS12T) ts12_scatter_kernel(const uint32_t* __restrict__ kin, const uint32_t* __restrict__ vin,
                                                             uint32_t* __restrict__ vout, int n_cap,
                                                             const uint32_t* __restrict__ n_dev, const uint32_t* __restrict__ table,
                                                             const uint32_t* __restrict__ totals, uint32_t* __restrict__ ranges, int T, int nbins) {
    __shared__ uint32_t cur[TS12_BINS];
    __shared__ uint16_t wcnt[TS12W][TS12_BINS];
    uint32_t* wtot = cur;
    constexpr int PERMAX = TS12_BINS / TS12T;
    constexpr int ROUNDS = TS12K / TS12T;
    const int per = nbins / TS12T;
    const int t = threadIdx.x, lane = t & 63, wave = t >> 6;
    const int n = n_dev ? (int)min((uint32_t)n_cap, n_dev[0]) : n_cap;
    if (blockIdx.x != 0 && (int)blockIdx.x >= ts12_blocks(n)) return;
    const int base = blockIdx.x * TS12K + wave * (64 * ROUNDS);
    const unsigned long long lt_mask = (lane == 0) ? 0ull : (~0ull >> (64 - lane));
    uint32_t ks[ROUNDS], vs[ROUNDS];
    uint16_t rk[ROUNDS];
#pragma unroll
    for (int c = 0; c < ROUNDS; c++) {
        const int e = base + c * 64 + lane;
        ks[c] = e < n ? kin[e] : 0u;
        vs[c] = e < n ? vin[e] : 0u;
    }
    uint32_t tot[PERMAX], pre[PERMAX];
    {
        const uint32_t* tp = totals + t * per;
        const uint32_t* rp = table + (size_t)blockIdx.x * nbins + t * per;
#pragma unroll
        for (int j = 0; j < PERMAX; j++) { tot[j] = j < per ? tp[j] : 0u; pre[j] = j < per ? rp[j] : 0u; }
    }
    uint32_t sum = 0;
#pragma unroll
    for (int j = 0; j < PERMAX; j++) sum += tot[j];
#pragma unroll
    for (int w = 0; w < TS12W; w++)
        for (int i = t; i < nbins / 2; i += TS12T) reinterpret_cast<uint32_t*>(&wcnt[w][0])[i] = 0u;
    uint32_t run = block_excl_scan<TS12W>(sum, wtot);
    __syncthreads();
#pragma unroll
    for (int j = 0; j < PERMAX; j++) {
        if (j < per) {
            const int tile = t * per + j;
            cur[tile] = run + pre[j];
            if (blockIdx.x == 0 && tile < T) {
                ranges[2 * tile] = tot[j] ? run : 0u;
                ranges[2 * tile + 1] = tot[j] ? run + tot[j] : 0u;
            }
            run += tot[j];
        }
    }
#pragma unroll
    for (int c = 0; c < ROUNDS; c++) {
        const bool valid = base + c * 64 + lane < n;
        const uint32_t d = ks[c] & (TS12_BINS - 1);
        const unsigned long long same = wave_match(d, 12, valid);
        const uint32_t in_round = (uint32_t)__popcll(same & lt_mask);
        const uint32_t prior = wcnt[wave][d];
        rk[c] = (uint16_t)(prior + in_round);
        if (valid && in_round == 0) wcnt[wave][d] = (uint16_t)(prior + (uint32_t)__popcll(same));
    }
    __syncthreads();
#pragma unroll
    for (int c = 0; c < ROUNDS; c++) {
        if (base + c * 64 + lane < n) {
            const uint32_t d = ks[c] & (TS12_BINS - 1);
            uint32_t pos = cur[d] + rk[c];
#pragma unroll
            for (int w = 0; w < TS12W - 1; w++)
                if (wave > w) pos += wcnt[w][d];
            vout[pos] = vs[c];
        }
    }
}

__global__ void __launch_bounds__(BLOCK) emit_kernel(int P, const uint32_t* __restrict__ order,
                                                     const uint32_t* __restrict__ tiles,
                                                     const uint32_t* __restrict__ offsets, float* __restrict__ rec,
                                                     const int32_t* __restrict__ radii, int gx, int gy,
                                                     uint32_t* __restrict__ tile_keys, uint32_t* __restrict__ vals,
                                                     uint32_t cap, uint32_t* __restrict__ ranges, int n_ranges,
                                                     uint32_t* __restrict__ seg_count, uint32_t* __restrict__ gtot,
                                                     int n_gtot, const uint32_t* __restrict__ span,
                                                     uint32_t* __restrict__ disp_ctr) {
    const int i = blockIdx.x * BLOCK + threadIdx.x;
    for (int j = i; j < n_ranges; j += gridDim.x * BLOCK) ranges[j] = 0u;
    for (int j = i; j < n_gtot; j += gridDim.x * BLOCK) gtot[j] = 0u;
    for (int j = i; j < DISP_CTR_WORDS; j += gridDim.x * BLOCK) disp_ctr[j] = 0u;
    if (i == 0) seg_count[0] = 0u;
    const int lane = threadIdx.x & 63;
    const uint32_t nvis = min((uint32_t)P, span[0]);
    if ((uint32_t)(i - lane) >= nvis) return;
    const bool valid = (uint32_t)i < nvis;
    const uint32_t g = valid ? order[i] : 0u;
    const uint32_t off = valid ? offsets[i] : 0u;
    const uint2 tr = valid ? reinterpret_cast<const uint2*>(tiles)[g] : make_uint2(0u, 0u);
    const uint32_t n = tr.x, rect = tr.y;
    if (n != 0u) {
        rec[(size_t)g * REC + R_IBASE] = __builtin_bit_cast(float, off);
        rec[(size_t)g * REC + R_RECT] = __builtin_bit_cast(float, rect);
    }
    const uint32_t incl = wave_incl_scan_u32(n);
    const uint32_t loc = incl - n;
    const uint32_t M = (uint32_t)__builtin_amdgcn_readlane((int)incl, 63);
    const uint32_t base = (uint32_t)__builtin_amdgcn_readfirstlane((int)(off - loc));
    for (uint32_t j0 = 0; j0 < M; j0 += 64u) {
        const uint32_t j = j0 + (uint32_t)lane;
        int lo = 0;
#pragma unroll
        for (int step = 32; step >= 1; step >>= 1) {
            const int mid = lo + step;
            const uint32_t v = (uint32_t)__builtin_amdgcn_ds_bpermute(mid << 2, (int)loc);
            lo = v <= j ? mid : lo;
        }
        const uint32_t t = j - (uint32_t)__builtin_amdgcn_ds_bpermute(lo << 2, (int)loc);
        const uint32_t go = (uint32_t)__builtin_amdgcn_ds_bpermute(lo << 2, (int)g);
        const uint32_t ro = (uint32_t)__builtin_amdgcn_ds_bpermute(lo << 2, (int)rect);
        const uint32_t w = max(ro >> 20, 1u), ty = t / w, tx = t - ty * w;
        const uint32_t pos = base + j;
        if (j < M && pos < cap) {
            tile_keys[pos] = (((ro >> 10) & 1023u) + ty) * (uint32_t)gx + ((ro & 1023u) + tx);
            vals[pos] = go;
        }
    }
}

__global__ void __launch_bounds__(BLOCK) ranges_kernel(int R_cap, const uint32_t* __restrict__ R_dev,
                                                       const uint32_t* __restrict__ tile_keys,
                                                       uint32_t* __restrict__ ranges) {
    const int i = blockIdx.x * BLOCK + threadIdx.x;
    const int R = R_dev ? (int)min((uint32_t)R_cap, R_dev[0]) : R_cap;
    if (i >= R) return;
    const uint32_t cur = tile_keys[i];
    if (i == 0) ranges[2 * cur] = 0;
    else {
        const uint32_t prev = tile_keys[i - 1];
        if (cur != prev) { ranges[2 * prev + 1] = (uint32_t)i; ranges[2 * cur] = (uint32_t)i; }
    }
    if (i == R - 1) ranges[2 * cur + 1] = (uint32_t)R;
}

__global__ void __launch_bounds__(1024) order_xcd_kernel(const uint32_t* __restrict__ counts, int n, uint32_t* __restrict__ order,
                                                         uint32_t* __restrict__ prefix, uint32_t* __restrict__ slot_prefix,
                                                         uint32_t* __restrict__ total, unsigned long long* __restrict__ host_total,
                                                         uint32_t host_tag, uint32_t cap_R, long long cap_slots, uint32_t magic, int gx,
                                                         int order_n) {
    __shared__ uint32_t hist[1024];
    __shared__ uint32_t wsum[16];
    __shared__ unsigned long long wsum2[16];
    __shared__ uint32_t wzero[16];
    const int t = threadIdx.x, lane = t & 63, wave = t >> 6;
    const uint32_t c = blockIdx.x;
    hist[t] = 0;
    auto both = [](uint32_t v) { return (unsigned long long)v | ((unsigned long long)seg_slots(v) << 32); };
    const int per = ((n + 7) / 8 + 1023) / 1024 * 1024;
    const int p0 = min(n, (int)c * per), p1 = min(n, p0 + per);
    __syncthreads();
    unsigned long long before = 0;
    uint32_t zeros = 0;
    for (int i = t; i < n; i += 1024) {
        const uint32_t len = counts[i];
        const int tile = i >> 2;
        if (xcd_of_tile(tile % gx, tile / gx) == c) atomicAdd(&hist[1023u - min(1023u, len)], 1u);
        if (i < p0) before += both(len);
        zeros += len == 0u ? 1u : 0u;
    }
    before = wave_reduce_add(before);
    zeros = wave_reduce_add(zeros);
    if (lane == 0) { wsum2[wave] = before; wzero[wave] = zeros; }
    __syncthreads();
    unsigned long long run = 0;
    uint32_t n_empty = 0;
#pragma unroll
    for (int w = 0; w < 16; w++) { run += wsum2[w]; n_empty += wzero[w]; }
    uint32_t n_mine;
    hist[t] = block_excl_scan<16>(hist[t], wsum, &n_mine);
    __syncthreads();
    for (int i0 = p0; i0 < p1; i0 += 1024) {
        const int i = i0 + t;
        const unsigned long long v = both(i < p1 ? counts[i] : 0u);
        const unsigned long long inc = (unsigned long long)wave_incl_scan_u32((uint32_t)v) | ((unsigned long long)wave_incl_scan_u32((uint32_t)(v >> 32)) << 32);
        __syncthreads();
        unsigned long long all;
        const unsigned long long ex = run + block_excl_scan<16>(v, inc, wsum2, &all);
        if (i < p1) {
            if (prefix) prefix[i] = (uint32_t)ex;
            if (slot_prefix) slot_prefix[i] = (uint32_t)(ex >> 32);
        }
        run += all;
    }
    if (c == 7 && t == 0) {
        if (total) {
            total[1] = (uint32_t)run; total[2] = (uint32_t)(run >> 32);
            total[3] = magic; total[4] = cap_R; total[5] = (uint32_t)(unsigned long long)cap_slots; total[6] = (uint32_t)((unsigned long long)cap_slots >> 32);
        }
        if (host_total) {
            __hip_atomic_store(host_total + 2, ((unsigned long long)host_tag << 32) | (unsigned long long)((uint32_t)n - n_empty), __ATOMIC_RELAXED, __HIP_MEMORY_SCOPE_SYSTEM);
            __hip_atomic_store(host_total, ((unsigned long long)host_tag << 32) | (run & 0xffffffffull), __ATOMIC_RELAXED, __HIP_MEMORY_SCOPE_SYSTEM);
            __hip_atomic_store(host_total + 1, ((unsigned long long)host_tag << 32) | (run >> 32), __ATOMIC_RELAXED, __HIP_MEMORY_SCOPE_SYSTEM);
        }
    }
    for (int i = t; i < n; i += 1024) {
        const int tile = i >> 2;
        if (xcd_of_tile(tile % gx, tile / gx) != c) continue;
        const uint32_t len = counts[i];
        order[8u * atomicAdd(&hist[1023u - min(1023u, len)], 1u) + c] = (uint32_t)i;
    }
    for (uint32_t j = n_mine + (uint32_t)t; 8u * j + c < (uint32_t)order_n; j += 1024u) order[8u * j + c] = ORDER_NONE;
}

}

void launch_order_desc(const uint32_t* counts, int n, uint32_t* order, uint32_t* prefix, uint32_t* slot_prefix, uint32_t* totals,
                       unsigned long long* host_totals, uint32_t host_tag, uint32_t cap_R, long long cap_slots, uint32_t magic, int gx, int order_n,
                       hipStream_t s) {
    hipLaunchKernelGGL(order_xcd_kernel, dim3(8), dim3(1024), 0, s, counts, n, order, prefix, slot_prefix, totals, host_totals,
                       host_tag, cap_R, cap_slots, magic, gx, order_n);
}

template <int ITEMS>
static void radix_sort_impl(uint32_t* const key[2], uint32_t* const val[2], int n, const uint32_t* n_dev, int total_bits,
                            int bits_per_pass, uint32_t* tbl, uint32_t* gtot, hipStream_t s, const RadixWeights* weights) {
    const int per = BLOCK * ITEMS;
    const int nb = (n + per - 1) / per;
    const int ng = (nb + GS - 1) / GS;
    const int passes = (total_bits + bits_per_pass - 1) / bits_per_pass;
    assert(!weights || (n_dev == nullptr && bits_per_pass <= 8 && passes <= RADIX_WGTOT_SLOT));
    for (int p = 0; p < passes; p++) {
        const int lo = p * bits_per_pass, nbits = std::min(bits_per_pass, total_bits - lo);
        uint32_t* gt = gtot + (size_t)p * ng * 256;
        if (weights && p == passes - 1) {
            const WeightArgs wa{val[p & 1], gtot + (size_t)RADIX_WGTOT_SLOT * ng * 256, *weights};
            hipLaunchKernelGGL((radix_hist_kernel<ITEMS, true>), dim3(nb), dim3(BLOCK), 0, s, key[p & 1], n, n_dev, lo,
                               (1u << nbits) - 1, tbl, gt, wa);
            hipLaunchKernelGGL((radix_scatter_kernel<ITEMS, true>), dim3(nb), dim3(BLOCK), 0, s, key[p & 1], val[p & 1],
                               key[(p + 1) & 1], val[(p + 1) & 1], n, n_dev, lo, nbits, tbl, gt, ng, wa);
            break;
        }
        hipLaunchKernelGGL((radix_hist_kernel<ITEMS>), dim3(nb), dim3(BLOCK), 0, s, key[p & 1], n, n_dev, lo,
                           (1u << nbits) - 1, tbl, gt, WeightArgs{});
        hipLaunchKernelGGL((radix_scatter_kernel<ITEMS>), dim3(nb), dim3(BLOCK), 0, s, key[p & 1], val[p & 1],
                           key[(p + 1) & 1], val[(p + 1) & 1], n, n_dev, lo, nbits, tbl, gt, ng, WeightArgs{});
    }
}

void launch_radix_sort(uint32_t* const key[2], uint32_t* const val[2], int n, const uint32_t* n_dev, int total_bits,
                       int bits_per_pass, uint32_t* table, hipStream_t s, const RadixWeights* weights) {
    if (n <= 0) return;
    uint32_t* gtot = radix_gtot(table, n);
    if (n <= (1 << 20)) radix_sort_impl<4>(key, val, n, n_dev, total_bits, bits_per_pass, table, gtot, s, weights);
    else radix_sort_impl<16>(key, val, n, n_dev, total_bits, bits_per_pass, table, gtot, s, weights);
}

void launch_depth_bucket_sort(uint32_t* const key[2], uint32_t* const val[2], int n, uint32_t* table, int cap, hipStream_t s, const RadixWeights& w) {
    if (n <= 0) return;
    constexpr int ITEMS = 4;
    assert(n <= DEPTH_BUCKET_MAX_P && cap >= DEPTH_BUCKET_CAP_MIN && cap <= DEPTH_BUCKET_CAP);
    const int nb = (n + BLOCK * ITEMS - 1) / (BLOCK * ITEMS), ng = (nb + GS - 1) / GS;
    uint32_t* gtot = radix_gtot(table, n);
    uint32_t* wgtot = gtot + (size_t)RADIX_WGTOT_SLOT * ng * 256;
    const WeightArgs wa{val[0], wgtot, w};
    hipLaunchKernelGGL((radix_hist_kernel<ITEMS, true, true>), dim3(nb), dim3(BLOCK), 0, s, key[0], n, (const uint32_t*)nullptr, 16, 255u, table, gtot, wa);
    hipLaunchKernelGGL((depth_bucket_scatter_kernel<ITEMS>), dim3(nb), dim3(BLOCK), 0, s, key[0], val[0], key[1], val[1], w.offsets, n, 16, table, gtot,
                       wgtot, ng, w);
    hipLaunchKernelGGL(depth_bucket_sort_kernel, dim3(256), dim3(DB_THREADS), 0, s, key[0], val[0], key[1], val[1], w.offsets, w.tiles, gtot, wgtot, ng, cap);
}

void launch_emit(int P, const uint32_t* order, const uint32_t* tiles, const uint32_t* offsets, float* rec,
                 const int32_t* radii, int gx, int gy, uint32_t* tile_keys, uint32_t* vals, int cap, uint32_t* ranges,
                 uint32_t* seg_count, uint32_t* sort_table, const uint32_t* span, uint32_t* disp_ctr, hipStream_t s) {
    hipLaunchKernelGGL(emit_kernel, dim3((P + BLOCK - 1) / BLOCK), dim3(BLOCK), 0, s, P, order, tiles, offsets, rec,
                       radii, gx, gy, tile_keys, vals, (uint32_t)cap, ranges, 2 * gx * gy + (gx * gy + 255) / 256 * SEG_BLOCK_STRIDE, seg_count,
                       radix_gtot(sort_table, cap), (int)radix_gtot_words(cap), span, disp_ctr);
}

void launch_tile_sort12(uint32_t* const key[2], uint32_t* const val[2], int n, const uint32_t* n_dev, uint32_t* table, uint32_t* ranges, int T,
                        hipStream_t s) {
    if (n <= 0) return;
    const int nb = ts12_blocks(n);
    const int nbins = (T + TS12T - 1) / TS12T * TS12T;
    uint32_t* totals = table + (size_t)nb * nbins;
    hipLaunchKernelGGL(ts12_hist_kernel, dim3(nb), dim3(TS12T), 0, s, key[0], n, n_dev, table, nbins);
    hipLaunchKernelGGL(ts12_colscan_kernel, dim3(nbins / 16), dim3(BLOCK), 0, s, table, nb, n, n_dev, totals, nbins);
    hipLaunchKernelGGL(ts12_scatter_kernel, dim3(nb), dim3(TS12T), 0, s, key[0], val[0], val[1], n, n_dev, table, totals, ranges, T, nbins);
}

void launch_ranges(int R, const uint32_t* R_dev, const uint32_t* tile_keys, uint32_t* ranges, int T, hipStream_t s) {
    if (R > 0) hipLaunchKernelGGL(ranges_kernel, dim3((R + BLOCK - 1) / BLOCK), dim3(BLOCK), 0, s, R, R_dev, tile_keys, ranges);
}

}
```

### svg-ir_amd/csrc/depth_sort_plan.hpp

```cpp
#pragma once
#include <cstdlib>
#include <cstring>

namespace svgir {

enum class DepthSortPlan { kLsd = 0, kBuckets = 1 };

constexpr int DEPTH_BUCKET_MAX_P = 1 << 19;
constexpr int DEPTH_BUCKET_CAP = 8192;
constexpr int DEPTH_BUCKET_CAP_MIN = 64;

inline bool depth_sort_forced_lsd(const char* env) { return env && std::strcmp(env, "lsd") == 0; }
inline int depth_bucket_cap(const char* env) {
    if (!env || !env[0]) return DEPTH_BUCKET_CAP;
    const long v = std::strtol(env, nullptr, 10);
    return v < DEPTH_BUCKET_CAP_MIN ? DEPTH_BUCKET_CAP_MIN : (v > DEPTH_BUCKET_CAP ? DEPTH_BUCKET_CAP : (int)v);
}

inline DepthSortPlan depth_sort_plan(int P, int spec_top, bool forced_lsd) {
    return (!forced_lsd && spec_top >= 0 && P > 0 && P <= DEPTH_BUCKET_MAX_P) ? DepthSortPlan::kBuckets : DepthSortPlan::kLsd;
}

#if defined(__HIPCC__)
void launch_depth_bucket_sort(uint32_t* const key[2], uint32_t* const val[2], int n, uint32_t* table, int cap, hipStream_t s, const RadixWeights& w);
#endif

}
```

### svg-ir_amd/csrc/preprocess.hip

```cpp
#include "common.hpp"
#include "shade_tables.hpp"

#pragma clang fp contract(off)

namespace svgir {

namespace {

struct Mat3 {
    float m[3][3];
};
__device__ __forceinline__ Mat3 mmul(const Mat3& A, const Mat3& B) {
    Mat3 r;
#pragma unroll
    for (int c = 0; c < 3; c++)
#pragma unroll
        for (int row = 0; row < 3; row++)
            r.m[c][row] = A.m[0][row] * B.m[c][0] + A.m[1][row] * B.m[c][1] + A.m[2][row] * B.m[c][2];
    return r;
}
__device__ __forceinline__ Mat3 mtr(const Mat3& A) {
    Mat3 r;
#pragma unroll
    for (int c = 0; c < 3; c++)
#pragma unroll
        for (int row = 0; row < 3; row++) r.m[c][row] = A.m[row][c];
    return r;
}
__device__ __forceinline__ float ndc2pix(float v, int S) { return (float)((((double)v + 1.0) * S - 1.0) * 0.5); }

__device__ __forceinline__ float normalize3(float* v) {
    const float mod = fmaxf(sqrtf(v[0] * v[0] + v[1] * v[1] + v[2] * v[2]), (float)0.00000001);
    v[0] /= mod; v[1] /= mod; v[2] /= mod;
    return mod;
}

__device__ __forceinline__ void tile_rect(float px, float py, int rad, int gx, int gy, int* rmin, int* rmax) {
    const float r = (float)rad;
    rmin[0] = min(gx, max(0, (int)((px - r) / TILE)));
    rmin[1] = min(gy, max(0, (int)((py - r) / TILE)));
    rmax[0] = min(gx, max(0, (int)((px + r + TILE - 1) / TILE)));
    rmax[1] = min(gy, max(0, (int)((py + r + TILE - 1) / TILE)));
}

__constant__ float kC2[5] = {1.0925484305920792f, -1.0925484305920792f, 0.31539156525252005f, -1.0925484305920792f,
                             0.5462742152960396f};
__constant__ float kC3[7] = {-0.5900435899266435f, 2.890611442640554f, -0.4570457994644658f, 0.3731763325901154f,
                             -0.4570457994644658f, 1.445305721320277f, -0.5900435899266435f};

__device__ __forceinline__ void load_sh(const PreArgs& a, int idx, float* sh) {
    const float* shp = a.shs + (size_t)idx * a.M * 3;
    if (a.M == 16 && (((size_t)a.shs) & 15) == 0) {
#pragma unroll
        for (int i = 0; i < 12; i++) {
            const float4 v = reinterpret_cast<const float4*>(shp)[i];
            sh[4 * i] = v.x; sh[4 * i + 1] = v.y; sh[4 * i + 2] = v.z; sh[4 * i + 3] = v.w;
        }
    } else {
        const int n = 3 * (a.D + 1) * (a.D + 1);
#pragma unroll
        for (int i = 0; i < 48; i++) sh[i] = i < n ? shp[i] : 0.f;
    }
}

__device__ __forceinline__ uint32_t sh_to_rgb(const PreArgs& a, const float* sh, const float* campos, const float* pos, float* rgb) {
    const float kC0 = 0.28209479177387814f, kC1 = 0.4886025119029199f;
    float dir[3] = {pos[0] - campos[0], pos[1] - campos[1], pos[2] - campos[2]};
    const float len = sqrtf(dir[0] * dir[0] + dir[1] * dir[1] + dir[2] * dir[2]);
    const float x = dir[0] / len, y = dir[1] / len, z = dir[2] / len;
    float res[3];
#pragma unroll
    for (int c = 0; c < 3; c++) res[c] = kC0 * sh[c];
    if (a.D > 0) {
#pragma unroll
        for (int c = 0; c < 3; c++) res[c] = res[c] - kC1 * y * sh[3 + c] + kC1 * z * sh[6 + c] - kC1 * x * sh[9 + c];
        if (a.D > 1) {
            const float xx = x * x, yy = y * y, zz = z * z, xy = x * y, yz = y * z, xz = x * z;
#pragma unroll
            for (int c = 0; c < 3; c++)
                res[c] = res[c] + kC2[0] * xy * sh[12 + c] + kC2[1] * yz * sh[15 + c] +
                         kC2[2] * (2.0f * zz - xx - yy) * sh[18 + c] + kC2[3] * xz * sh[21 + c] +
                         kC2[4] * (xx - yy) * sh[24 + c];
            if (a.D > 2) {
#pragma unroll
                for (int c = 0; c < 3; c++)
                    res[c] = res[c] + kC3[0] * y * (3.0f * xx - yy) * sh[27 + c] + kC3[1] * xy * z * sh[30 + c] +
                             kC3[2] * y * (4.0f * zz - xx - yy) * sh[33 + c] +
                             kC3[3] * z * (2.0f * zz - 3.0f * xx - 3.0f * yy) * sh[36 + c] +
                             kC3[4] * x * (4.0f * zz - xx - yy) * sh[39 + c] + kC3[5] * z * (xx - yy) * sh[42 + c] +
                             kC3[6] * x * (xx - 3.0f * yy) * sh[45 + c];
            }
        }
    }
    uint32_t mask = 0;
#pragma unroll
    for (int c = 0; c < 3; c++) {
        res[c] += 0.5f;
        if (res[c] < 0) mask |= 1u << c;
        rgb[c] = fmaxf(res[c], 0.0f);
    }
    return mask;
}

template <bool SVGSS>
__global__ void __launch_bounds__(BLOCK) preprocess_kernel(const PreArgs a) {
    const int idx = blockIdx.x * BLOCK + threadIdx.x;
    float V[16], PM[16], campos[3] = {0.f, 0.f, 0.f}, pbb[4] = {0.f, 0.f, 0.f, 0.f};
#pragma unroll
    for (int i = 0; i < 16; i++) { V[i] = a.view[i]; PM[i] = a.proj[i]; }
    if (!a.colors_precomp) { campos[0] = a.campos[0]; campos[1] = a.campos[1]; campos[2] = a.campos[2]; }
    if (SVGSS) { pbb[0] = a.patchbbox[0]; pbb[1] = a.patchbbox[1]; pbb[2] = a.patchbbox[2]; pbb[3] = a.patchbbox[3]; }
    for (int j = idx; j < a.n_zero_words; j += gridDim.x * BLOCK) a.zero_words[j] = 0u;
    if ((int)blockIdx.x >= a.pblocks) {
        shade_table_entry(a.tabs, ((int)blockIdx.x - a.pblocks) * BLOCK + (int)threadIdx.x);
        return;
    }
    if (idx >= a.P) return;
    const bool surface = cfg_flag(a.cfg, 0), pix_depth = cfg_flag(a.cfg, 2);
    if (a.out_weights) a.out_weights[idx] = 0.f;
    if (a.needed) a.needed[idx] = 0;
    if (idx == 0 && a.span) *a.span = 0u;
    a.radii[idx] = 0;
    a.tiles[2 * idx] = 0;
    a.key[idx] = a.spec_top >= 0 ? (((uint32_t)a.spec_top << 24) | 0x00FFFFFFu) : 0xFFFFFFFFu;
    a.idx[idx] = (uint32_t)idx;
    if ((threadIdx.x & 63) == 0) a.key_top[idx >> 6] = 0xff00u;

    const float po[3] = {a.means3D[3 * idx], a.means3D[3 * idx + 1], a.means3D[3 * idx + 2]};
    float q[4] = {1.f, 0.f, 0.f, 0.f};
    if (a.rotations) {
        const float4 qq = reinterpret_cast<const float4*>(a.rotations)[idx];
        q[0] = qq.x; q[1] = qq.y; q[2] = qq.z; q[3] = qq.w;
    }
    const float hx = PM[0] * po[0] + PM[4] * po[1] + PM[8] * po[2] + PM[12];
    const float hy = PM[1] * po[0] + PM[5] * po[1] + PM[9] * po[2] + PM[13];
    const float hw = PM[3] * po[0] + PM[7] * po[1] + PM[11] * po[2] + PM[15];
    const float pw = 1.0f / (hw + 0.0000001f);
    const float ppx = hx * pw, ppy = hy * pw;
    const float pv[3] = {V[0] * po[0] + V[4] * po[1] + V[8] * po[2] + V[12],
                         V[1] * po[0] + V[5] * po[1] + V[9] * po[2] + V[13],
                         V[2] * po[0] + V[6] * po[1] + V[10] * po[2] + V[14]};
    const float pix[2] = {ndc2pix(ppx, a.W), ndc2pix(ppy, a.H)};
    if (SVGSS) {
        const float x0 = pbb[1], y0 = pbb[0], x1 = pbb[3], y1 = pbb[2];
        const float w = x1 - x0, h = y1 - y0, e = (float)0.2;
        if (pv[2] < 0 || pix[0] < x0 - w * e || pix[0] >= x1 + w * e || pix[1] < y0 - h * e || pix[1] >= y1 + h * e) {
            if (a.prefilter_violation) *a.prefilter_violation = 1u;
            return;
        }
    } else {
        if (pv[2] <= 0.2f) {
            if (a.prefilter_violation) *a.prefilter_violation = 1u;
            return;
        }
    }

    const float r = q[0], x = q[1], y = q[2], z = q[3];
    Mat3 Rm;
    Rm.m[0][0] = 1.f - 2.f * (y * y + z * z); Rm.m[0][1] = 2.f * (x * y - r * z); Rm.m[0][2] = 2.f * (x * z + r * y);
    Rm.m[1][0] = 2.f * (x * y + r * z); Rm.m[1][1] = 1.f - 2.f * (x * x + z * z); Rm.m[1][2] = 2.f * (y * z - r * x);
    Rm.m[2][0] = 2.f * (x * z - r * y); Rm.m[2][1] = 2.f * (y * z + r * x); Rm.m[2][2] = 1.f - 2.f * (x * x + y * y);

    float nv[3] = {0, 0, 0}, J[10];
#pragma unroll
    for (int i = 0; i < 10; i++) J[i] = 0;
    if (surface) {
        const float nw[3] = {Rm.m[0][2], Rm.m[1][2], Rm.m[2][2]};
        const float a0w[3] = {Rm.m[0][0], Rm.m[1][0], Rm.m[2][0]};
        const float a1w[3] = {Rm.m[0][1], Rm.m[1][1], Rm.m[2][1]};
        float a0[3], a1[3];
#pragma unroll
        for (int i = 0; i < 3; i++) {
            nv[i] = V[i] * nw[0] + V[4 + i] * nw[1] + V[8 + i] * nw[2];
            a0[i] = V[i] * a0w[0] + V[4 + i] * a0w[1] + V[8 + i] * a0w[2];
            a1[i] = V[i] * a1w[0] + V[4 + i] * a1w[1] + V[8 + i] * a1w[2];
        }
        const float dot = pv[0] * nv[0] + pv[1] * nv[1] + pv[2] * nv[2];
        if ((double)dot > -0.01) {
            if (a.prefilter_violation) *a.prefilter_violation = 1u;
            return;
        }
        if (pix_depth) {
            const float qx = pv[0] / pv[2], qy = pv[1] / pv[2];
            const float S_fix = 1000, Svp = (a.focal_x + a.focal_y) / 2;
            float d0[3] = {qx + 1 / S_fix, qy, 1};
            const float m0 = normalize3(d0);
            float d1[3] = {qx, qy + 1 / S_fix, 1};
            const float m1 = normalize3(d1);
            const float c0 = d0[0] * nv[0] + d0[1] * nv[1] + d0[2] * nv[2];
            const float c1 = d1[0] * nv[0] + d1[1] * nv[1] + d1[2] * nv[2];
            if (fabsf(c0 / m0) < 0.01f || fabsf(c1 / m1) < 0.01f) return;
            const float t = pv[0] * nv[0] + pv[1] * nv[1] + pv[2] * nv[2];
            const float t0 = t / c0, t1 = t / c1;
            float xu0[3], xu1[3];
#pragma unroll
            for (int i = 0; i < 3; i++) { xu0[i] = d0[i] * t0 - pv[i]; xu1[i] = d1[i] * t1 - pv[i]; }
            const float k = Svp / S_fix;
            J[0] = (xu0[0] * a0[0] + xu0[1] * a0[1] + xu0[2] * a0[2]) / k;
            J[1] = (xu1[0] * a0[0] + xu1[1] * a0[1] + xu1[2] * a0[2]) / k;
            J[2] = (xu0[0] * a1[0] + xu0[1] * a1[1] + xu0[2] * a1[2]) / k;
            J[3] = (xu1[0] * a1[0] + xu1[1] * a1[1] + xu1[2] * a1[2]) / k;
#pragma unroll
            for (int i = 0; i < 3; i++) { J[4 + i] = a0[i]; J[7 + i] = a1[i]; }
        }
    }

    float sc_in[3] = {0.f, 0.f, 0.f}, c3[6], rgb[3] = {0.f, 0.f, 0.f}, sh[48];
    if (a.scales) { sc_in[0] = a.scales[3 * idx]; sc_in[1] = a.scales[3 * idx + 1]; sc_in[2] = a.scales[3 * idx + 2]; }
    if (a.cov3D_precomp) {
#pragma unroll
        for (int i = 0; i < 6; i++) c3[i] = a.cov3D_precomp[6 * idx + i];
    }
    const float opacity = a.opacities[idx];
    if (a.colors_precomp) {
#pragma unroll
        for (int c = 0; c < 3; c++) rgb[c] = a.colors_precomp[3 * idx + c];
    } else {
        load_sh(a, idx, sh);
    }
    if (!a.cov3D_precomp) {
        Mat3 Sm;
#pragma unroll
        for (int c = 0; c < 3; c++)
#pragma unroll
            for (int rr = 0; rr < 3; rr++) Sm.m[c][rr] = 0.f;
        Sm.m[0][0] = a.scale_modifier * sc_in[0];
        Sm.m[1][1] = a.scale_modifier * sc_in[1];
        Sm.m[2][2] = (a.scale_modifier * (surface ? 1.0f : 0.0f)) != 0.0f ? 0.0f : sc_in[2];
        const Mat3 Mm = mmul(Sm, Rm);
        const Mat3 Sg = mmul(mtr(Mm), Mm);
        c3[0] = Sg.m[0][0]; c3[1] = Sg.m[0][1]; c3[2] = Sg.m[0][2];
        c3[3] = Sg.m[1][1]; c3[4] = Sg.m[1][2]; c3[5] = Sg.m[2][2];
#pragma unroll
        for (int i = 0; i < 6; i++) a.cov3D[6 * idx + i] = c3[i];
    }

    float t[3] = {pv[0], pv[1], pv[2]};
    const float limx = 1.3f * a.tanx, limy = 1.3f * a.tany;
    const float txtz = t[0] / t[2], tytz = t[1] / t[2];
    t[0] = fminf(limx, fmaxf(-limx, txtz)) * t[2];
    t[1] = fminf(limy, fmaxf(-limy, tytz)) * t[2];
    Mat3 Jm, Wm, Vk;
    Jm.m[0][0] = a.focal_x / t[2]; Jm.m[0][1] = 0.f; Jm.m[0][2] = -(a.focal_x * t[0]) / (t[2] * t[2]);
    Jm.m[1][0] = 0.f; Jm.m[1][1] = a.focal_y / t[2]; Jm.m[1][2] = -(a.focal_y * t[1]) / (t[2] * t[2]);
    Jm.m[2][0] = 0.f; Jm.m[2][1] = 0.f; Jm.m[2][2] = 0.f;
    Wm.m[0][0] = V[0]; Wm.m[0][1] = V[4]; Wm.m[0][2] = V[8];
    Wm.m[1][0] = V[1]; Wm.m[1][1] = V[5]; Wm.m[1][2] = V[9];
    Wm.m[2][0] = V[2]; Wm.m[2][1] = V[6]; Wm.m[2][2] = V[10];
    Vk.m[0][0] = c3[0]; Vk.m[0][1] = c3[1]; Vk.m[0][2] = c3[2];
    Vk.m[1][0] = c3[1]; Vk.m[1][1] = c3[3]; Vk.m[1][2] = c3[4];
    Vk.m[2][0] = c3[2]; Vk.m[2][1] = c3[4]; Vk.m[2][2] = c3[5];
    const Mat3 Tm = mmul(Wm, Jm);
    const Mat3 cov = mmul(mmul(mtr(Tm), mtr(Vk)), Tm);
    const float ca = cov.m[0][0] + 0.3f, cb = cov.m[0][1], cc = cov.m[1][1] + 0.3f;
    const float det = ca * cc - cb * cb;
    if (det == 0.0f) return;
    const float det_inv = 1.f / det;
    const float conic[3] = {cc * det_inv, -cb * det_inv, ca * det_inv};
    const float mid = 0.5f * (ca + cc);
    const float l1 = mid + sqrtf(fmaxf(0.1f, mid * mid - det));
    const float l2 = mid - sqrtf(fmaxf(0.1f, mid * mid - det));
    const float my_radius = ceilf(3.f * sqrtf(fmaxf(l1, l2)));
    int rmin[2], rmax[2];
    tile_rect(pix[0], pix[1], (int)my_radius, a.gx, a.gy, rmin, rmax);
    const int area = (rmax[0] - rmin[0]) * (rmax[1] - rmin[1]);
    if (area == 0) return;

    float emb[5] = {0.f, 0.f, 0.f, 0.f, 0.f};
    if (a.embed_S > 0) {
#pragma unroll
        for (int ch = 0; ch < 5; ch++) emb[ch] = ch < a.embed_S ? a.features[(size_t)idx * a.embed_S + ch] : 0.f;
    }
    uint32_t cmask = 0;
    if (!a.colors_precomp) cmask = sh_to_rgb(a, sh, campos, po, rgb);
    a.clamped[idx] = cmask;
    a.radii[idx] = (int)my_radius;
    reinterpret_cast<uint2*>(a.tiles)[idx] = make_uint2((uint32_t)area, (uint32_t)rmin[0] | ((uint32_t)rmin[1] << 10) | ((uint32_t)(rmax[0] - rmin[0]) << 20));
    const uint32_t depth_key = __float_as_uint(pv[2]);
    a.key[idx] = depth_key;
    {
        const unsigned long long act = __ballot(true);
        uint32_t av = 0, ov = 0;
#pragma unroll
        for (int b = 0; b < 8; b++) {
            const unsigned long long m = __ballot((depth_key >> (24 + b)) & 1u);
            av |= (m == act) ? (1u << b) : 0u;
            ov |= (m != 0ull) ? (1u << b) : 0u;
        }
        if ((threadIdx.x & 63) == (unsigned)(__ffsll((long long)act) - 1)) a.key_top[idx >> 6] = (av << 8) | ov;
    }

    float iu = 0.f, iv = 0.f;
    if (SVGSS) {
        const float umx = (float)(0.5 * (double)sc_in[0] + 0.1);
        const float umy = (float)(0.5 * (double)sc_in[1] + 0.1);
        iu = 1.0f / umx; iv = 1.0f / umy;
    }
    float4* rec = reinterpret_cast<float4*>(a.rec + (size_t)idx * REC);
    rec[0] = make_float4(pix[0], pix[1], conic[0], conic[1]);
    const float da = J[0] * J[6] + J[2] * J[9], db = J[1] * J[6] + J[3] * J[9];
    rec[1] = make_float4(conic[2], opacity, pv[2], da);
    const bool embed = a.embed_S > 0;
    rec[2] = embed ? make_float4(emb[0], emb[1], emb[2], emb[3]) : make_float4(J[0], J[1], J[2], J[3]);
    rec[3] = make_float4(db, rgb[0], rgb[1], rgb[2]);
    rec[4] = make_float4(nv[0], nv[1], nv[2], embed ? emb[4] : iu);
    rec[5] = make_float4(iv, 0.f, 0.f, 0.f);
}

__global__ void __launch_bounds__(BLOCK) mark_visible_kernel(int P, const float* means3D, const float* V,
                                                             uint8_t* present) {
    const int idx = blockIdx.x * BLOCK + threadIdx.x;
    if (idx >= P) return;
    const float z = V[2] * means3D[3 * idx] + V[6] * means3D[3 * idx + 1] + V[10] * means3D[3 * idx + 2] + V[14];
    present[idx] = z <= 0.2f ? 0 : 1;
}

}

void launch_preprocess(const PreArgs& a_, bool svgss, hipStream_t s) {
    PreArgs a = a_;
    a.pblocks = (a.P + BLOCK - 1) / BLOCK;
    const int grid = a.pblocks + (a.tabs.entries() + BLOCK - 1) / BLOCK;
    if (svgss) hipLaunchKernelGGL(preprocess_kernel<true>, dim3(grid), dim3(BLOCK), 0, s, a);
    else hipLaunchKernelGGL(preprocess_kernel<false>, dim3(grid), dim3(BLOCK), 0, s, a);
}

void launch_mark_visible(int P, const float* means3D, const float* view, uint8_t* present, hipStream_t s) {
    hipLaunchKernelGGL(mark_visible_kernel, dim3((P + BLOCK - 1) / BLOCK), dim3(BLOCK), 0, s, P, means3D, view, present);
}

}
```

Measured before the change: 668.0 million surfels/s.

## Fuse depth-bucket histogram and scatter into preprocess via per-row bucket plan

On the bucket depth-sort path, preprocess now runs 1024-thread blocks that rank visible surfels by their top depth byte within the block. Each block writes a per-row sorted segment along with count and weight prefix tables, so the separate histogram and scatter kernels are removed. The bucket sort kernel then gathers each bucket's items from all rows using a binary search over the row prefixes, and it writes the culled ids itself. This saves global passes and kernel launches over keys and ids. The cost is larger preprocess blocks, with possible occupancy or register pressure, and indirect gathers with a binary search per item in the sort kernel.

```diff
diff --git a/svg-ir_amd/csrc/api.hip b/svg-ir_amd/csrc/api.hip
--- a/svg-ir_amd/csrc/api.hip
+++ b/svg-ir_amd/csrc/api.hip
@@ -420,6 +420,11 @@
     return n;
 }
 
+static_assert(DEPTH_ROW == 1024, "a row of the bucket plan = a sort block: sort_blocks() sizes the row tables");
+inline DepthRows geom_depth_rows(const GeomLayout& g, int P) {
+    return DepthRows{g.key[0], g.idx[0], g.shade_list, g.radix_tbl, g.radix_wtbl, radix_gtot(g.radix_tbl, P)};
+}
+
 struct ForwardCall {
     const svgir_view_call c; const svgir_params* p = c.params; const svgir_outputs* o = c.outputs; hipStream_t s = (hipStream_t)c.stream;
     bool key_spec;
@@ -556,26 +561,29 @@
         pa.needed = prepass ? G.needed : nullptr;
         pa.span = G.counters + 3;
         if (p->shade) pa.tabs = shade_tables(&p->shade->sp, nullptr, 0);
-        pa.zero_words = radix_gtot(G.radix_tbl, P); pa.n_zero_words = (int)radix_gtot_words(P);
         ckey = workload_key(p);
         static const bool key_spec_env = getenv("SVGIR_NO_KEY_SPEC") == nullptr;
         spec_top = (key_spec && key_spec_env) ? g_history.guess_top(ckey) : -1;
         pa.spec_top = spec_top; pa.key_top = G.key_top;
+        static const bool forced_lsd = depth_sort_forced_lsd(getenv("SVGIR_DEPTH_SORT"));
+        static const int bucket_cap = depth_bucket_cap(getenv("SVGIR_DEPTH_BUCKET_CAP"));
+        const bool buckets = depth_sort_plan(P, spec_top, forced_lsd) == DepthSortPlan::kBuckets;
+        const DepthRows rows = geom_depth_rows(G, P);
+        pa.zero_words = radix_gtot(G.radix_tbl, P); pa.n_zero_words = (int)radix_gtot_words(P);
         pa.prefilter_violation = nullptr;
         if (p->prefiltered) {
             HIP_OK(hipMemsetAsync(G.counters, 0, 16, s));
             pa.prefilter_violation = G.counters + 1;
         }
-        launch_preprocess(pa, svgss, s);
+        if (buckets) launch_preprocess_rows(pa, rows, svgss, s);
+        else launch_preprocess(pa, svgss, s);
         if (int rc = check("preprocess")) return rc;
         stage_mark(tm, "preprocess");
 
         const int depth_bits = spec_top >= 0 ? 24 : 32;
         depth_order = G.idx[(depth_bits / 8) & 1];
         const RadixWeights rw{G.tiles, G.radix_wtbl, G.offsets, G.counters, G.key_top, (P + 63) / 64, pa.prefilter_violation, R_pin.at, R_pin.tag};
-        static const bool forced_lsd = depth_sort_forced_lsd(getenv("SVGIR_DEPTH_SORT"));
-        static const int bucket_cap = depth_bucket_cap(getenv("SVGIR_DEPTH_BUCKET_CAP"));
-        if (depth_sort_plan(P, spec_top, forced_lsd) == DepthSortPlan::kBuckets) launch_depth_bucket_sort(G.key, G.idx, P, G.radix_tbl, bucket_cap, s, rw);
+        if (buckets) launch_depth_bucket_sort(rows, G.key[1], G.idx[1], P, bucket_cap, s, rw);
         else launch_radix_sort(G.key, G.idx, P, nullptr, depth_bits, 8, G.radix_tbl, s, &rw);
         if (int rc = check("depth sort")) return rc;
         stage_mark(tm, "sort_depth");
diff --git a/svg-ir_amd/csrc/binning.hip b/svg-ir_amd/csrc/binning.hip
--- a/svg-ir_amd/csrc/binning.hip
+++ b/svg-ir_amd/csrc/binning.hip
@@ -18,7 +18,7 @@
     RadixWeights w;
 };
 
-template <int ITEMS, bool W = false, bool F = false>
+template <int ITEMS, bool W = false>
 __global__ void __launch_bounds__(BLOCK) radix_hist_kernel(const uint32_t* __restrict__ keys, int n_cap,
                                                            const uint32_t* __restrict__ n_dev, int bit_lo,
                                                            uint32_t mask, uint32_t* __restrict__ table,
@@ -44,8 +44,7 @@
 #pragma unroll
     for (int i = 0; i < ITEMS; i++) {
         const int e = base + i * BLOCK + threadIdx.x;
-        if constexpr (F) { if (e < n && w[i] != 0u) atomicAdd(&hist[(k[i] >> bit_lo) & mask], 1u); }
-        else if (e < n) atomicAdd(&hist[(k[i] >> bit_lo) & mask], 1u);
+        if (e < n) atomicAdd(&hist[(k[i] >> bit_lo) & mask], 1u);
         if constexpr (W) if (e < n && w[i] != 0u) atomicAdd(&whist[(k[i] >> bit_lo) & mask], w[i]);
     }
     __syncthreads();
@@ -54,7 +53,7 @@
     if (c) atomicAdd(&gtot[(size_t)(blockIdx.x / GS) * 256 + threadIdx.x], c);
     if constexpr (W) {
         const uint32_t wc = whist[threadIdx.x];
-        if constexpr (!F) wa.w.wtable[(size_t)blockIdx.x * 256 + threadIdx.x] = wc;
+        wa.w.wtable[(size_t)blockIdx.x * 256 + threadIdx.x] = wc;
         if (wc) atomicAdd(&wa.wgtot[(size_t)(blockIdx.x / GS) * 256 + threadIdx.x], wc);
     }
 }
@@ -247,104 +246,6 @@
 }
 
 
-template <int ITEMS>
-__global__ void __launch_bounds__(BLOCK) depth_bucket_scatter_kernel(const uint32_t* __restrict__ kin, const uint32_t* __restrict__ vin,
-                                                                     uint32_t* __restrict__ kout, uint32_t* __restrict__ vout,
-                                                                     uint32_t* __restrict__ wout, int n, int bit_lo,
-                                                                     const uint32_t* __restrict__ table, const uint32_t* __restrict__ gtot,
-                                                                     const uint32_t* __restrict__ wgtot, int ngroups, RadixWeights w) {
-    __shared__ uint32_t wcnt[4][256];
-    __shared__ uint32_t wtot[4], wtot2[4], wtot3[4], ksum[4], wcul[4];
-    const int t = threadIdx.x, lane = t & 63, wave = t >> 6;
-    const int base = blockIdx.x * (BLOCK * ITEMS) + wave * (64 * ITEMS);
-    const unsigned long long lt_mask = (lane == 0) ? 0ull : (~0ull >> (64 - lane));
-    uint32_t ks[ITEMS], vs[ITEMS], ws[ITEMS], rk[ITEMS];
-#pragma unroll
-    for (int c = 0; c < ITEMS; c++) {
-        const int e = base + c * 64 + lane;
-        ks[c] = e < n ? kin[e] : 0u;
-        vs[c] = e < n ? vin[e] : 0u;
-    }
-#pragma unroll
-    for (int c = 0; c < ITEMS; c++) ws[c] = base + c * 64 + lane < n ? w.tiles[2 * (size_t)vs[c]] : 0u;
-    if (blockIdx.x == 0) {
-        uint32_t kv = 0xff00u;
-#pragma unroll 8
-        for (int j = t; j < w.n_key_top; j += BLOCK) kv = key_top_fold(kv, w.key_top[j]);
-        kv = wave_reduce(kv, key_top_fold);
-        if (lane == 0) ksum[wave] = kv;
-    }
-#pragma unroll
-    for (int q = 0; q < 4; q++) wcnt[q][t] = 0;
-    uint32_t cursor, nvis, cull_base;
-    {
-        const int g = blockIdx.x / GS;
-        uint32_t tot = 0, pre = 0, wsum = 0;
-#pragma unroll 8
-        for (int gg = 0; gg < ngroups; gg++) {
-            const uint32_t v = gtot[(size_t)gg * 256 + t];
-            tot += v;
-            pre += gg < g ? v : 0u;
-            if (blockIdx.x == 0) wsum += wgtot[(size_t)gg * 256 + t];
-        }
-#pragma unroll 8
-        for (int b = g * GS; b < (int)blockIdx.x; b++) pre += table[(size_t)b * 256 + t];
-        cursor = block_excl_scan<4>(tot, wtot, &nvis) + pre;
-        cull_base = nvis + blockIdx.x * (BLOCK * ITEMS) - block_sum<4>(pre, wtot3);
-        if (blockIdx.x == 0) {
-            uint32_t R;
-            (void)block_excl_scan<4>(wsum, wtot2, &R);
-            if (t == 0) {
-                const uint32_t summary = key_top_fold(key_top_fold(ksum[0], ksum[1]), key_top_fold(ksum[2], ksum[3]));
-                w.counters[0] = R;
-                w.counters[2] = summary;
-                w.counters[3] = nvis;
-                if (w.host_out) {
-                    const uint32_t viol = w.violation ? (w.violation[0] != 0u ? 1u : 0u) : 0u;
-                    __hip_atomic_store(w.host_out, ((unsigned long long)w.host_tag << 32) | R, __ATOMIC_RELAXED, __HIP_MEMORY_SCOPE_SYSTEM);
-                    __hip_atomic_store(w.host_out + 1, ((unsigned long long)w.host_tag << 32) | (viol << 16) | summary, __ATOMIC_RELAXED,
-                                       __HIP_MEMORY_SCOPE_SYSTEM);
-                }
-            }
-        }
-    }
-    uint32_t ncul = 0;
-#pragma unroll
-    for (int c = 0; c < ITEMS; c++) {
-        const bool valid = base + c * 64 + lane < n && ws[c] != 0u;
-        const uint32_t d = (ks[c] >> bit_lo) & 255u;
-        const unsigned long long same = wave_match(d, 8, valid);
-        const uint32_t in_round = (uint32_t)__popcll(same & lt_mask);
-        const uint32_t prior = wcnt[wave][d];
-        rk[c] = prior + in_round;
-        if (valid && in_round == 0) wcnt[wave][d] = prior + (uint32_t)__popcll(same);
-        const unsigned long long culled = __ballot(base + c * 64 + lane < n && ws[c] == 0u);
-        if (!valid) rk[c] = ncul + (uint32_t)__popcll(culled & lt_mask);
-        ncul += (uint32_t)__popcll(culled);
-    }
-    if (lane == 0) wcul[wave] = ncul;
-    __syncthreads();
-    {
-        const uint32_t c0 = wcnt[0][t], c1 = wcnt[1][t], c2 = wcnt[2][t];
-        __syncthreads();
-        wcnt[0][t] = cursor; wcnt[1][t] = cursor + c0; wcnt[2][t] = cursor + c0 + c1; wcnt[3][t] = cursor + c0 + c1 + c2;
-    }
-    __syncthreads();
-    for (int q = 0; q < wave; q++) cull_base += wcul[q];
-#pragma unroll
-    for (int c = 0; c < ITEMS; c++) {
-        if (base + c * 64 + lane >= n) continue;
-        if (ws[c] != 0u) {
-            const uint32_t pos = wcnt[wave][(ks[c] >> bit_lo) & 255u] + rk[c];
-            kout[pos] = ks[c];
-            vout[pos] = vs[c];
-            wout[pos] = ws[c];
-        } else {
-            vout[cull_base + rk[c]] = vs[c];
-        }
-    }
-}
-
 constexpr int DB_THREADS = 1024, DB_WAVES = DB_THREADS / 64, DB_ROUNDS = DEPTH_BUCKET_CAP / DB_THREADS;
 
 template <bool CARRY, class Get, class Put>
@@ -394,28 +295,84 @@
     __syncthreads();
 }
 
-__global__ void __launch_bounds__(DB_THREADS) depth_bucket_sort_kernel(uint32_t* key0, uint32_t* val0, uint32_t* key1, uint32_t* val1, uint32_t* offsets,
-                                                                       const uint32_t* __restrict__ tiles, const uint32_t* __restrict__ gtot,
-                                                                       const uint32_t* __restrict__ wgtot, int ngroups, int cap) {
+__device__ __forceinline__ int bucket_row_of(const uint32_t* prefix, int nrows, uint32_t j) {
+    int lo = 0, hi = nrows;
+    while (hi - lo > 1) {
+        const int mid = (lo + hi) >> 1;
+        if (prefix[mid] <= j) lo = mid; else hi = mid;
+    }
+    return lo;
+}
+
+__global__ void __launch_bounds__(DB_THREADS) depth_bucket_sort_kernel(const DepthRows rows, int nrows, int P, uint32_t* key1, uint32_t* val1,
+                                                                       uint32_t* offsets, int cap, const RadixWeights w) {
     __shared__ uint32_t sA[DEPTH_BUCKET_CAP], sB[DEPTH_BUCKET_CAP], sI[DEPTH_BUCKET_CAP], sW[DEPTH_BUCKET_CAP];
     __shared__ uint32_t wcnt[DB_WAVES][256];
-    __shared__ uint32_t cur[256], wsum[DB_WAVES], wsum2[DB_WAVES], hdr[3], red[2][DB_WAVES];
+    __shared__ uint32_t cur[256], wsum[DB_WAVES], wsum2[DB_WAVES], tot3[3][DB_WAVES], ksum[DB_WAVES], red[2][DB_WAVES];
+    static_assert(3 * (DEPTH_ROWS_MAX + 1) <= DEPTH_BUCKET_CAP && DEPTH_ROWS_MAX <= DB_THREADS, "row prefixes: one row per thread, inside sB");
+    static_assert(sizeof(uint32_t) * (4 * DEPTH_BUCKET_CAP + DB_WAVES * 256 + 256 + 8 * DB_WAVES) <= 160 * 1024, "LDS of one CU");
+    uint32_t* const prefix = sB;
+    uint32_t* const rowsrc = sB + (DEPTH_ROWS_MAX + 1);
+    uint32_t* const vprefix = sB + 2 * (DEPTH_ROWS_MAX + 1);
     const int t = threadIdx.x, lane = t & 63, wave = t >> 6;
-    uint32_t cnt = 0, wt = 0;
-    if (t < 256)
-        for (int g = 0; g < ngroups; g++) { cnt += gtot[(size_t)g * 256 + t]; wt += wgtot[(size_t)g * 256 + t]; }
-    const uint32_t cpre = block_excl_scan<DB_WAVES>(cnt, wsum);
-    const uint32_t wpre = block_excl_scan<DB_WAVES>(wt, wsum2);
-    if (t == (int)blockIdx.x) { hdr[0] = cpre; hdr[1] = cnt; hdr[2] = wpre; }
-    __syncthreads();
-    const uint32_t start = hdr[0], wbase = hdr[2];
-    const int n = (int)hdr[1];
+    const uint32_t d = blockIdx.x;
+    uint32_t c0 = 0, c1 = 0, w0 = 0;
+    uint2 rt = make_uint2(0u, 0u);
+    if (t < nrows) {
+        rt = reinterpret_cast<const uint2*>(rows.tot)[t];
+        c0 = rows.cscan[(size_t)t * 256 + d];
+        c1 = d < 255u ? rows.cscan[(size_t)t * 256 + d + 1] : rt.x;
+        w0 = rows.wscan[(size_t)t * 256 + d];
+    }
+    uint32_t kv = 0xff00u;
+    if (d == 0u) {
+#pragma unroll 4
+        for (int j = t; j < w.n_key_top; j += DB_THREADS) kv = key_top_fold(kv, w.key_top[j]);
+    }
+    uint32_t n_u, V;
+    const uint32_t pre = block_excl_scan<DB_WAVES>(c1 - c0, wsum, &n_u);
+    const uint32_t vpre = block_excl_scan<DB_WAVES>(rt.x, wsum2, &V);
+    {
+        const uint32_t s0 = wave_reduce_add(c0), s1 = wave_reduce_add(w0), s2 = wave_reduce_add(rt.y);
+        kv = wave_reduce(kv, key_top_fold);
+        if (lane == 0) { tot3[0][wave] = s0; tot3[1][wave] = s1; tot3[2][wave] = s2; ksum[wave] = kv; }
+    }
+    if (t < nrows) { prefix[t] = pre; rowsrc[t] = (uint32_t)t * DEPTH_ROW + c0 - pre; vprefix[t] = vpre; }
+    if (t == nrows) { prefix[t] = n_u; vprefix[t] = V; }
+    if (t == 0 && nrows == DB_THREADS) { prefix[nrows] = n_u; vprefix[nrows] = V; }
+    __syncthreads();
+    uint32_t start = 0, wbase = 0, R = 0;
+#pragma unroll
+    for (int q = 0; q < DB_WAVES; q++) { start += tot3[0][q]; wbase += tot3[1][q]; R += tot3[2][q]; }
+    const int n = (int)n_u;
+    if (d == 0u && t == 0) {
+        uint32_t summary = 0xff00u;
+#pragma unroll
+        for (int q = 0; q < DB_WAVES; q++) summary = key_top_fold(summary, ksum[q]);
+        w.counters[0] = R;
+        w.counters[2] = summary;
+        w.counters[3] = V;
+        if (w.host_out) {
+            const uint32_t viol = w.violation ? (w.violation[0] != 0u ? 1u : 0u) : 0u;
+            __hip_atomic_store(w.host_out, ((unsigned long long)w.host_tag << 32) | R, __ATOMIC_RELAXED, __HIP_MEMORY_SCOPE_SYSTEM);
+            __hip_atomic_store(w.host_out + 1, ((unsigned long long)w.host_tag << 32) | (viol << 16) | summary, __ATOMIC_RELAXED,
+                               __HIP_MEMORY_SCOPE_SYSTEM);
+        }
+    }
+    for (int b = (int)d; b < nrows; b += 256) {
+        const uint32_t vb = vprefix[b], nv = vprefix[b + 1] - vb;
+        const int len = min(DEPTH_ROW, P - b * DEPTH_ROW) - (int)nv;
+        const uint32_t* src = rows.id + (size_t)b * DEPTH_ROW + nv;
+        uint32_t* dst = val1 + V + ((uint32_t)b * DEPTH_ROW - vb);
+        for (int i = t; i < len; i += DB_THREADS) dst[i] = src[i];
+    }
     if (n == 0) return;
     if (n <= cap) {
         for (int i = t; i < n; i += DB_THREADS) {
-            sA[i] = (key1[start + i] << 16) | (uint32_t)i;
-            sI[i] = val1[start + i];
-            sW[i] = offsets[start + i];
+            const uint32_t src = rowsrc[bucket_row_of(prefix, nrows, (uint32_t)i)] + (uint32_t)i;
+            sA[i] = (rows.key[src] << 16) | (uint32_t)i;
+            sI[i] = rows.id[src];
+            sW[i] = rows.w[src];
         }
         bucket_pass<false>(n, 16, [&](int i) { return make_uint2(sA[i], 0u); }, [&](uint32_t pos, uint2 it) { sB[pos] = it.x; }, wcnt, cur, wsum);
         bucket_pass<false>(n, 24, [&](int i) { return make_uint2(sB[i], 0u); }, [&](uint32_t pos, uint2 it) { sA[pos] = it.x; }, wcnt, cur, wsum);
@@ -440,9 +397,13 @@
         }
         return;
     }
+    const auto item = [&](int i) {
+        const uint32_t src = rowsrc[bucket_row_of(prefix, nrows, (uint32_t)i)] + (uint32_t)i;
+        return make_uint2(rows.key[src], rows.id[src]);
+    };
     {
         uint32_t a = 0xffffu, o = 0u;
-        for (int i = t; i < n; i += DB_THREADS) { const uint32_t k = key1[start + i] & 0xffffu; a &= k; o |= k; }
+        for (int i = t; i < n; i += DB_THREADS) { const uint32_t k = item(i).x & 0xffffu; a &= k; o |= k; }
         a = wave_reduce(a, [](uint32_t x, uint32_t y) { return x & y; });
         o = wave_reduce(o, [](uint32_t x, uint32_t y) { return x | y; });
         if (lane == 0) { red[0][wave] = a; red[1][wave] = o; }
@@ -450,24 +411,33 @@
         a = 0xffffu; o = 0u;
 #pragma unroll
         for (int q = 0; q < DB_WAVES; q++) { a &= red[0][q]; o |= red[1][q]; }
-        if (a != o) {
+        if (a == o) {
+            for (int i = t; i < n; i += DB_THREADS) val1[start + i] = item(i).y;
+        } else {
+            uint32_t* const tk = offsets + start;
+            uint32_t* const tv = key1 + start;
             for (int pass = 0; pass < 2; pass++) {
-                const uint32_t* sk = (pass ? key0 : key1) + start; const uint32_t* sv = (pass ? val0 : val1) + start;
-                uint32_t* dk = (pass ? key1 : key0) + start; uint32_t* dv = (pass ? val1 : val0) + start;
                 const int shift = 8 * pass;
                 if (t < 256) cur[t] = 0u;
                 __syncthreads();
-                for (int i = t; i < n; i += DB_THREADS) atomicAdd(&cur[(sk[i] >> shift) & 255u], 1u);
+                for (int i = t; i < n; i += DB_THREADS) atomicAdd(&cur[((pass ? tk[i] : item(i).x) >> shift) & 255u], 1u);
                 __syncthreads();
                 const uint32_t ex = block_excl_scan<DB_WAVES>(t < 256 ? cur[t] : 0u, wsum);
                 if (t < 256) cur[t] = ex;
-                for (int c0 = 0; c0 < n; c0 += cap)
-                    bucket_pass<true>(min(cap, n - c0), shift, [&](int i) { return make_uint2(sk[c0 + i], sv[c0 + i]); },
-                                      [&](uint32_t pos, uint2 it) { dk[pos] = it.x; dv[pos] = it.y; }, wcnt, cur, wsum);
+                for (int c0 = 0; c0 < n; c0 += cap) {
+                    if (pass == 0)
+                        bucket_pass<true>(min(cap, n - c0), shift, [&](int i) { return item(c0 + i); },
+                                          [&](uint32_t pos, uint2 it) { tk[pos] = it.x; tv[pos] = it.y; }, wcnt, cur, wsum);
+                    else
+                        bucket_pass<true>(min(cap, n - c0), shift, [&](int i) { return make_uint2(tk[c0 + i], tv[c0 + i]); },
+                                          [&](uint32_t pos, uint2 it) { val1[start + pos] = it.y; }, wcnt, cur, wsum);
+                }
                 __threadfence_block();
                 __syncthreads();
             }
         }
+        __threadfence_block();
+        __syncthreads();
     }
     uint32_t carry = wbase;
     for (int c0 = 0; c0 < n; c0 += DB_THREADS * DB_ROUNDS) {
@@ -475,7 +445,7 @@
 #pragma unroll
         for (int j = 0; j < DB_ROUNDS; j++) {
             const int i = c0 + t * DB_ROUNDS + j;
-            wv[j] = i < n ? tiles[2 * (size_t)val1[start + i]] : 0u;
+            wv[j] = i < n ? w.tiles[2 * (size_t)val1[start + i]] : 0u;
             sum += wv[j];
         }
         uint32_t all;
@@ -804,18 +774,10 @@
     else radix_sort_impl<16>(key, val, n, n_dev, total_bits, bits_per_pass, table, gtot, s, weights);
 }
 
-void launch_depth_bucket_sort(uint32_t* const key[2], uint32_t* const val[2], int n, uint32_t* table, int cap, hipStream_t s, const RadixWeights& w) {
+void launch_depth_bucket_sort(const DepthRows& rows, uint32_t* key1, uint32_t* val1, int n, int cap, hipStream_t s, const RadixWeights& w) {
     if (n <= 0) return;
-    constexpr int ITEMS = 4;
     assert(n <= DEPTH_BUCKET_MAX_P && cap >= DEPTH_BUCKET_CAP_MIN && cap <= DEPTH_BUCKET_CAP);
-    const int nb = (n + BLOCK * ITEMS - 1) / (BLOCK * ITEMS), ng = (nb + GS - 1) / GS;
-    uint32_t* gtot = radix_gtot(table, n);
-    uint32_t* wgtot = gtot + (size_t)RADIX_WGTOT_SLOT * ng * 256;
-    const WeightArgs wa{val[0], wgtot, w};
-    hipLaunchKernelGGL((radix_hist_kernel<ITEMS, true, true>), dim3(nb), dim3(BLOCK), 0, s, key[0], n, (const uint32_t*)nullptr, 16, 255u, table, gtot, wa);
-    hipLaunchKernelGGL((depth_bucket_scatter_kernel<ITEMS>), dim3(nb), dim3(BLOCK), 0, s, key[0], val[0], key[1], val[1], w.offsets, n, 16, table, gtot,
-                       wgtot, ng, w);
-    hipLaunchKernelGGL(depth_bucket_sort_kernel, dim3(256), dim3(DB_THREADS), 0, s, key[0], val[0], key[1], val[1], w.offsets, w.tiles, gtot, wgtot, ng, cap);
+    hipLaunchKernelGGL(depth_bucket_sort_kernel, dim3(256), dim3(DB_THREADS), 0, s, rows, depth_rows(n), n, key1, val1, w.offsets, cap, w);
 }
 
 void launch_emit(int P, const uint32_t* order, const uint32_t* tiles, const uint32_t* offsets, float* rec,
diff --git a/svg-ir_amd/csrc/depth_sort_plan.hpp b/svg-ir_amd/csrc/depth_sort_plan.hpp
--- a/svg-ir_amd/csrc/depth_sort_plan.hpp
+++ b/svg-ir_amd/csrc/depth_sort_plan.hpp
@@ -1,4 +1,5 @@
 #pragma once
+#include <cstdint>
 #include <cstdlib>
 #include <cstring>
 
@@ -9,6 +10,9 @@
 constexpr int DEPTH_BUCKET_MAX_P = 1 << 19;
 constexpr int DEPTH_BUCKET_CAP = 8192;
 constexpr int DEPTH_BUCKET_CAP_MIN = 64;
+constexpr int DEPTH_ROW = 1024;
+constexpr int DEPTH_ROWS_MAX = DEPTH_BUCKET_MAX_P / DEPTH_ROW;
+inline int depth_rows(int P) { return (P + DEPTH_ROW - 1) / DEPTH_ROW; }
 
 inline bool depth_sort_forced_lsd(const char* env) { return env && std::strcmp(env, "lsd") == 0; }
 inline int depth_bucket_cap(const char* env) {
@@ -21,8 +25,16 @@
     return (!forced_lsd && spec_top >= 0 && P > 0 && P <= DEPTH_BUCKET_MAX_P) ? DepthSortPlan::kBuckets : DepthSortPlan::kLsd;
 }
 
+struct DepthRows {
+    uint32_t *key, *id, *w;
+    uint32_t* cscan;
+    uint32_t* wscan;
+    uint32_t* tot;
+};
+
 #if defined(__HIPCC__)
-void launch_depth_bucket_sort(uint32_t* const key[2], uint32_t* const val[2], int n, uint32_t* table, int cap, hipStream_t s, const RadixWeights& w);
+void launch_preprocess_rows(const PreArgs& a, const DepthRows& rows, bool svgss, hipStream_t s);
+void launch_depth_bucket_sort(const DepthRows& rows, uint32_t* key1, uint32_t* val1, int n, int cap, hipStream_t s, const RadixWeights& w);
 #endif
 
 }
diff --git a/svg-ir_amd/csrc/preprocess.hip b/svg-ir_amd/csrc/preprocess.hip
--- a/svg-ir_amd/csrc/preprocess.hip
+++ b/svg-ir_amd/csrc/preprocess.hip
@@ -1,4 +1,5 @@
 #include "common.hpp"
+#include "depth_sort_plan.hpp"
 #include "shade_tables.hpp"
 
 #pragma clang fp contract(off)
@@ -102,8 +103,9 @@
     return mask;
 }
 
-template <bool SVGSS>
-__global__ void __launch_bounds__(BLOCK) preprocess_kernel(const PreArgs a) {
+template <bool SVGSS, bool BK>
+__global__ void __launch_bounds__(BK ? DEPTH_ROW : BLOCK) preprocess_kernel(const PreArgs a, const DepthRows rows) {
+    constexpr int BLOCK = BK ? DEPTH_ROW : svgir::BLOCK;
     const int idx = blockIdx.x * BLOCK + threadIdx.x;
     float V[16], PM[16], campos[3] = {0.f, 0.f, 0.f}, pbb[4] = {0.f, 0.f, 0.f, 0.f};
 #pragma unroll
@@ -115,15 +117,19 @@
         shade_table_entry(a.tabs, ((int)blockIdx.x - a.pblocks) * BLOCK + (int)threadIdx.x);
         return;
     }
-    if (idx >= a.P) return;
+    uint32_t vis_key = 0u, vis_w = 0u;
+    const bool visible = [&]() -> bool {
+    if (idx >= a.P) return false;
     const bool surface = cfg_flag(a.cfg, 0), pix_depth = cfg_flag(a.cfg, 2);
     if (a.out_weights) a.out_weights[idx] = 0.f;
     if (a.needed) a.needed[idx] = 0;
     if (idx == 0 && a.span) *a.span = 0u;
     a.radii[idx] = 0;
     a.tiles[2 * idx] = 0;
-    a.key[idx] = a.spec_top >= 0 ? (((uint32_t)a.spec_top << 24) | 0x00FFFFFFu) : 0xFFFFFFFFu;
-    a.idx[idx] = (uint32_t)idx;
+    if constexpr (!BK) {
+        a.key[idx] = a.spec_top >= 0 ? (((uint32_t)a.spec_top << 24) | 0x00FFFFFFu) : 0xFFFFFFFFu;
+        a.idx[idx] = (uint32_t)idx;
+    }
     if ((threadIdx.x & 63) == 0) a.key_top[idx >> 6] = 0xff00u;
 
     const float po[3] = {a.means3D[3 * idx], a.means3D[3 * idx + 1], a.means3D[3 * idx + 2]};
@@ -146,12 +152,12 @@
         const float w = x1 - x0, h = y1 - y0, e = (float)0.2;
         if (pv[2] < 0 || pix[0] < x0 - w * e || pix[0] >= x1 + w * e || pix[1] < y0 - h * e || pix[1] >= y1 + h * e) {
             if (a.prefilter_violation) *a.prefilter_violation = 1u;
-            return;
+            return false;
         }
     } else {
         if (pv[2] <= 0.2f) {
             if (a.prefilter_violation) *a.prefilter_violation = 1u;
-            return;
+            return false;
         }
     }
 
@@ -178,7 +184,7 @@
         const float dot = pv[0] * nv[0] + pv[1] * nv[1] + pv[2] * nv[2];
         if ((double)dot > -0.01) {
             if (a.prefilter_violation) *a.prefilter_violation = 1u;
-            return;
+            return false;
         }
         if (pix_depth) {
             const float qx = pv[0] / pv[2], qy = pv[1] / pv[2];
@@ -189,7 +195,7 @@
             const float m1 = normalize3(d1);
             const float c0 = d0[0] * nv[0] + d0[1] * nv[1] + d0[2] * nv[2];
             const float c1 = d1[0] * nv[0] + d1[1] * nv[1] + d1[2] * nv[2];
-            if (fabsf(c0 / m0) < 0.01f || fabsf(c1 / m1) < 0.01f) return;
+            if (fabsf(c0 / m0) < 0.01f || fabsf(c1 / m1) < 0.01f) return false;
             const float t = pv[0] * nv[0] + pv[1] * nv[1] + pv[2] * nv[2];
             const float t0 = t / c0, t1 = t / c1;
             float xu0[3], xu1[3];
@@ -254,7 +260,7 @@
     const Mat3 cov = mmul(mmul(mtr(Tm), mtr(Vk)), Tm);
     const float ca = cov.m[0][0] + 0.3f, cb = cov.m[0][1], cc = cov.m[1][1] + 0.3f;
     const float det = ca * cc - cb * cb;
-    if (det == 0.0f) return;
+    if (det == 0.0f) return false;
     const float det_inv = 1.f / det;
     const float conic[3] = {cc * det_inv, -cb * det_inv, ca * det_inv};
     const float mid = 0.5f * (ca + cc);
@@ -264,7 +270,7 @@
     int rmin[2], rmax[2];
     tile_rect(pix[0], pix[1], (int)my_radius, a.gx, a.gy, rmin, rmax);
     const int area = (rmax[0] - rmin[0]) * (rmax[1] - rmin[1]);
-    if (area == 0) return;
+    if (area == 0) return false;
 
     float emb[5] = {0.f, 0.f, 0.f, 0.f, 0.f};
     if (a.embed_S > 0) {
@@ -277,7 +283,8 @@
     a.radii[idx] = (int)my_radius;
     reinterpret_cast<uint2*>(a.tiles)[idx] = make_uint2((uint32_t)area, (uint32_t)rmin[0] | ((uint32_t)rmin[1] << 10) | ((uint32_t)(rmax[0] - rmin[0]) << 20));
     const uint32_t depth_key = __float_as_uint(pv[2]);
-    a.key[idx] = depth_key;
+    if constexpr (BK) { vis_key = depth_key; vis_w = (uint32_t)area; }
+    else a.key[idx] = depth_key;
     {
         const unsigned long long act = __ballot(true);
         uint32_t av = 0, ov = 0;
@@ -305,6 +312,56 @@
     rec[3] = make_float4(db, rgb[0], rgb[1], rgb[2]);
     rec[4] = make_float4(nv[0], nv[1], nv[2], embed ? emb[4] : iu);
     rec[5] = make_float4(iv, 0.f, 0.f, 0.f);
+    return true;
+    }();
+    if constexpr (BK) {
+        constexpr int WAVES = BLOCK / 64;
+        __shared__ uint32_t wcnt[WAVES][256];
+        __shared__ uint32_t whist[256], wsum[WAVES], wsum2[WAVES], wcul[WAVES];
+        const int t = threadIdx.x, lane = t & 63, wave = t >> 6;
+        const unsigned long long lt_mask = (lane == 0) ? 0ull : (~0ull >> (64 - lane));
+        for (int i = t; i < WAVES * 256; i += BLOCK) (&wcnt[0][0])[i] = 0u;
+        if (t < 256) whist[t] = 0u;
+        __syncthreads();
+        const uint32_t d = (vis_key >> 16) & 255u;
+        const unsigned long long same = wave_match(d, 8, visible);
+        uint32_t rk = (uint32_t)__popcll(same & lt_mask);
+        if (visible) {
+            if (rk == 0) wcnt[wave][d] = (uint32_t)__popcll(same);
+            atomicAdd(&whist[d], vis_w);
+        }
+        const bool other = !visible && idx < a.P;
+        const unsigned long long others = __ballot(other);
+        if (other) rk = (uint32_t)__popcll(others & lt_mask);
+        if (lane == 0) wcul[wave] = (uint32_t)__popcll(others);
+        __syncthreads();
+        uint32_t c[WAVES], total = 0, wt = 0;
+#pragma unroll
+        for (int q = 0; q < WAVES; q++) { c[q] = t < 256 ? wcnt[q][t] : 0u; total += c[q]; }
+        if (t < 256) wt = whist[t];
+        uint32_t nvis, wall;
+        uint32_t run = block_excl_scan<WAVES>(total, wsum, &nvis);
+        const uint32_t wrun = block_excl_scan<WAVES>(wt, wsum2, &wall);
+        const size_t row = blockIdx.x;
+        if (t < 256) {
+            rows.cscan[row * 256 + t] = run;
+            rows.wscan[row * 256 + t] = wrun;
+#pragma unroll
+            for (int q = 0; q < WAVES; q++) { wcnt[q][t] = run; run += c[q]; }
+        }
+        if (t == 0) reinterpret_cast<uint2*>(rows.tot)[row] = make_uint2(nvis, wall);
+        __syncthreads();
+        if (visible) {
+            const size_t pos = row * BLOCK + wcnt[wave][d] + rk;
+            rows.key[pos] = vis_key;
+            rows.id[pos] = (uint32_t)idx;
+            rows.w[pos] = vis_w;
+        } else if (other) {
+            uint32_t before = nvis;
+            for (int q = 0; q < wave; q++) before += wcul[q];
+            rows.id[row * BLOCK + before + rk] = (uint32_t)idx;
+        }
+    }
 }
 
 __global__ void __launch_bounds__(BLOCK) mark_visible_kernel(int P, const float* means3D, const float* V,
@@ -317,13 +374,21 @@
 
 }
 
-void launch_preprocess(const PreArgs& a_, bool svgss, hipStream_t s) {
+static void launch_pre(const PreArgs& a_, const DepthRows* rows, bool svgss, hipStream_t s) {
     PreArgs a = a_;
-    a.pblocks = (a.P + BLOCK - 1) / BLOCK;
-    const int grid = a.pblocks + (a.tabs.entries() + BLOCK - 1) / BLOCK;
-    if (svgss) hipLaunchKernelGGL(preprocess_kernel<true>, dim3(grid), dim3(BLOCK), 0, s, a);
-    else hipLaunchKernelGGL(preprocess_kernel<false>, dim3(grid), dim3(BLOCK), 0, s, a);
-}
+    const int block = rows ? DEPTH_ROW : BLOCK;
+    a.pblocks = (a.P + block - 1) / block;
+    const int grid = a.pblocks + (a.tabs.entries() + block - 1) / block;
+    if (rows) {
+        a.n_zero_words = 0;
+        if (svgss) hipLaunchKernelGGL((preprocess_kernel<true, true>), dim3(grid), dim3(block), 0, s, a, *rows);
+        else hipLaunchKernelGGL((preprocess_kernel<false, true>), dim3(grid), dim3(block), 0, s, a, *rows);
+    } else if (svgss) hipLaunchKernelGGL((preprocess_kernel<true, false>), dim3(grid), dim3(block), 0, s, a, DepthRows{});
+    else hipLaunchKernelGGL((preprocess_kernel<false, false>), dim3(grid), dim3(block), 0, s, a, DepthRows{});
+}
+
+void launch_preprocess(const PreArgs& a, bool svgss, hipStream_t s) { launch_pre(a, nullptr, svgss, s); }
+void launch_preprocess_rows(const PreArgs& a, const DepthRows& rows, bool svgss, hipStream_t s) { launch_pre(a, &rows, svgss, s); }
 
 void launch_mark_visible(int P, const float* means3D, const float* view, uint8_t* present, hipStream_t s) {
     hipLaunchKernelGGL(mark_visible_kernel, dim3((P + BLOCK - 1) / BLOCK), dim3(BLOCK), 0, s, P, means3D, view, present);
```

Measured after the change: 691.1 million surfels/s (median of 6 runs). 3.5% higher.
